# VladimirRadenkovic/Image-inpainting-and-Super-Resolution-using-Diffusion-Models-and-Conditional-Flow-Matching

Hardware: AMD Instinct MI355X
Metric: sampled images/sec (50-step, 32x32) (higher is better)
Workload: dtype bf16

## Files before the change

### image-inpainting-and-super-resolution-using-diffusion-models-and-conditional-flow-matching_amd/csrc/capi.hip

```cpp
#include <cstring>
#include <vector>

#include "capi_internal.h"

static thread_local std::string g_err;
void mi355_set_error(const std::string& msg) { g_err = msg; }

const mi355_debug_config& mi355_default_debug() {
  static const mi355_debug_config d = [] { mi355_debug_config c; mi355_debug_defaults(&c); return c; }();
  return d;
}

extern "C" {

int mi355_version(void) { return 108; }
void mi355_debug_defaults(mi355_debug_config* c) {
  if (!c) return;
  std::memset(c, 0, sizeof(*c));
  c->conv_ws = 1; c->conv_small = 15; c->conv_min_wgs = 512; c->conv_stagger = 0; c->conv_ablate = 0; c->conv_spin_limit = 1 << 22;
  c->conv_time_reps = 0; c->gn_apply_max_hw = 64; c->gn_fuse = 1; c->l2_warm = 1; c->attn_fused = 1; c->gn_epilogue = 7; c->conv_pp = 109; c->conv_edge = 15;
}
int mi355_unet_status(mi355_unet* net, int clear) {
  if (!net) { mi355_set_error("null handle"); return -1; }
  return unet_status(net, clear);
}
const char* mi355_last_error(void) { return g_err.c_str(); }

int mi355_unet_param_count(const mi355_unet_config* cfg) {
  if (!cfg) { mi355_set_error("null config"); return -1; }
  std::vector<ParamInfo> p;
  int rc = unet_enumerate_params(*cfg, p);
  return rc ? rc : (int)p.size();
}

int mi355_unet_param_info(const mi355_unet_config* cfg, int index, char* name, int name_cap, int64_t shape[4], int* ndim) {
  if (!cfg || !name || !shape || !ndim) { mi355_set_error("null argument"); return -1; }
  std::vector<ParamInfo> p;
  if (int rc = unet_enumerate_params(*cfg, p)) return rc;
  MI355_REQUIRE(index >= 0 && index < (int)p.size(), -1, "param index out of range");
  MI355_REQUIRE((int)p[index].name.size() + 1 <= name_cap, -1, "name buffer too small");
  std::strcpy(name, p[index].name.c_str());
  *ndim = (int)p[index].shape.size();
  for (int i = 0; i < 4; ++i) shape[i] = i < *ndim ? p[index].shape[i] : 1;
  return 0;
}

int64_t mi355_unet_weight_bytes(const mi355_unet_config* cfg) {
  if (!cfg) { mi355_set_error("null config"); return -1; }
  return unet_weight_bytes(*cfg);
}

int mi355_unet_create(const mi355_unet_config* cfg, const float* const* params_host, int n_params, void* dev_weights,
                      int64_t dev_weights_bytes, void* stream, mi355_unet** out) {
  if (!cfg) { mi355_set_error("null config"); return -1; }
  return unet_build(*cfg, params_host, n_params, dev_weights, dev_weights_bytes, S(stream), out);
}

void mi355_unet_destroy(mi355_unet* net) { delete net; }

int mi355_unet_forward(mi355_unet* net, const float* x, int x_channels, const float* cond, int cond_channels, const float* t,
                       float* out, int batch, void* workspace, int64_t workspace_bytes, void* stream) {
  return unet_forward(net, x, x_channels, cond, cond_channels, t, out, batch, workspace, workspace_bytes, S(stream));
}

int mi355_unet_forward_t(mi355_unet* net, const float* x, int x_channels, const float* cond, int cond_channels, float t, float* out,
                         int batch, void* workspace, int64_t workspace_bytes, void* stream) {
  MI355_REQUIRE(net && workspace && batch > 0, -1, "unet_forward_t: bad argument");
  const WsLayout l = unet_ws_layout(net, batch);
  MI355_REQUIRE((int64_t)l.total <= workspace_bytes, -2, "unet_forward_t: workspace too small");
  float* tdev = reinterpret_cast<float*>(reinterpret_cast<char*>(workspace) + l.emb2);
  if (int rc = fill_launch(tdev, t, 1, S(stream))) return rc;
  return unet_forward(net, x, x_channels, cond, cond_channels, tdev, out, batch, workspace, workspace_bytes, S(stream), uniform_t_run());
}

int mi355_unet_forward_labels(mi355_unet* net, const float* x, int x_channels, const float* cond, int cond_channels, const float* t, float t_host,
                              const int32_t* labels, float* out, int batch, void* workspace, int64_t workspace_bytes, void* stream) {
  MI355_REQUIRE(net && workspace && batch > 0, -1, "unet_forward_labels: bad argument");
  MI355_REQUIRE(!labels || net->num_classes > 0, -1, "unet_forward_labels: class labels given to a net built without num_classes");
  UnetRun run;
  run.labels = labels;
  if (!t) {
    const WsLayout l = unet_ws_layout(net, batch);
    MI355_REQUIRE((int64_t)l.total <= workspace_bytes, -2, "unet_forward_labels: workspace too small");
    float* tdev = reinterpret_cast<float*>(reinterpret_cast<char*>(workspace) + l.emb2);
    if (int rc = fill_launch(tdev, t_host, 1, S(stream))) return rc;
    t = tdev;
    run.t_uniform = 1;
  }
  return unet_forward(net, x, x_channels, cond, cond_channels, t, out, batch, workspace, workspace_bytes, S(stream), run);
}

int mi355_unet_vjp(mi355_unet* net, const float* grad_out, float* grad_x, int x_channels, int batch, void* workspace, int64_t workspace_bytes,
                   void* stream) {
  MI355_REQUIRE(net && workspace, -1, "unet_vjp: null argument");
  const int64_t engine_bytes = unet_workspace_bytes(net, batch);
  MI355_REQUIRE(workspace_bytes >= engine_bytes, -2, "unet_vjp: workspace too small");
  return unet_backward(net, grad_out, grad_x, x_channels, batch, workspace, workspace_bytes, S(stream));
}

int mi355_unet_plan_op(const mi355_unet* net, int index, int32_t fields[16]) {
  MI355_REQUIRE(net && fields, -1, "plan_op: null argument");
  if (index < 0 || index >= (int)net->ops.size()) return -1;
  const PlanOp& o = net->ops[index];
  const int32_t v[16] = {o.kind, o.src0, o.src1, o.dst, o.mode, o.ks, o.Cout, o.use_pro, o.pro_silu, o.res, o.res_mode, o.gn_site, o.heads, o.ch,
                         o.dst >= 0 ? net->tensors[o.dst].C : 0, o.dst >= 0 ? net->tensors[o.dst].H : 0};
  for (int i = 0; i < 16; ++i) fields[i] = v[i];
  return (int)net->ops.size();
}

int mi355_unet_read_tensor(const mi355_unet* net, int tensor, int gradient, float* out, int batch, void* workspace, int64_t workspace_bytes,
                           void* stream) {
  MI355_REQUIRE(net && out && workspace, -1, "read_tensor: null argument");
  MI355_REQUIRE(tensor >= 0 && tensor < (int)net->tensors.size(), -1, "read_tensor: tensor index out of range");
  MI355_REQUIRE(!gradient || net->cfg.differentiable, -4, "read_tensor: gradients exist in differentiable plans only");
  const WsView v(net, workspace, batch);
  MI355_REQUIRE((int64_t)v.l.total <= workspace_bytes, -2, "read_tensor: workspace too small");
  const PlanTensor& t = net->tensors[tensor];
  const int tstate = (!gradient && (size_t)tensor < net->tensor_state_n) ? (int)net->tensor_state[tensor].load(std::memory_order_relaxed) : 0;
  if (tstate) {
    mi355_set_error(tstate == 1
                        ? "read_tensor: the last forward did not materialise this tensor (a conv output whose only reader, a GroupNorm site, ran in the conv's "
                          "epilogue; a 1x1 skip conv that rode in the next 3x3 conv; the packed network input the first conv read from the caller's tensor): "
                          "create the handle with debug.gn_epilogue = 0, conv_small = 7, conv_edge = 3 to inspect it"
                        : "read_tensor: the last forward normalised this conv output in place (16x16 level: it holds silu(GroupNorm(.)), not the conv's result): "
                          "create the handle with debug.gn_epilogue = 0 (or 1) to inspect it");
    return MI355_ERR_UNSUPPORTED;
  }
  return unpack_nchw_launch(net->cfg.dtype, gradient ? v.grad(tensor) : v.tensor(tensor), batch, t.H * t.W, t.C, out, S(stream));
}

int mi355_unet_get_stats(const mi355_unet* net, int batch, mi355_unet_stats* out) {
  if (!net || !out) { mi355_set_error("null argument"); return -1; }
  out->launches = net->last_launches > 0 ? net->last_launches : net->launches;
  out->conv_flops = net->conv_flops * batch;
  out->attn_flops = net->attn_flops * batch;
  out->act_bytes = net->act_bytes * batch;
  out->weight_bytes = net->weight_bytes;
  return 0;
}

int mi355_unet_profile(mi355_unet* net, const float* x, int x_channels, const float* cond, int cond_channels, const float* t,
                       float* out, int batch, void* workspace, int64_t workspace_bytes, void* stream, mi355_op_profile* recs,
                       int cap) {
  MI355_REQUIRE(net && recs && cap > 0, -1, "unet_profile: bad argument");
  std::vector<mi355_op_profile> prof;
  std::vector<hipEvent_t> ev;
  UnetRun run; run.prof = &prof; run.prof_events = &ev;
  int rc = unet_forward(net, x, x_channels, cond, cond_channels, t, out, batch, workspace, workspace_bytes, S(stream), run);
  constexpr int NCAL = 17;
  hipEvent_t cal[NCAL];
  for (int i = 0; i < NCAL; ++i) { (void)hipEventCreate(&cal[i]); (void)hipEventRecord(cal[i], S(stream)); }
  hipError_t e = hipStreamSynchronize(S(stream));
  if (rc == 0 && e == hipSuccess) {
    float gap = 0.f;
    for (int i = 0; i + 1 < NCAL; ++i) { float ms = 0.f; (void)hipEventElapsedTime(&ms, cal[i], cal[i + 1]); gap += ms; }
    gap /= (float)(NCAL - 1);
    for (size_t i = 0; i + 1 < ev.size() && i < prof.size(); ++i) {
      float ms = 0.f;
      (void)hipEventElapsedTime(&ms, ev[i], ev[i + 1]);
      prof[i].ms = ms > 2.f * gap ? ms - gap : 0.5f * ms;
    }
  }
  for (int i = 0; i < NCAL; ++i) (void)hipEventDestroy(cal[i]);
  for (auto h : ev) (void)hipEventDestroy(h);
  if (rc) return rc;
  if (e != hipSuccess) { mi355_set_error(hipGetErrorString(e)); return -3; }
  const int n = (int)prof.size();
  for (int i = 0; i < n && i < cap; ++i) recs[i] = prof[i];
  return n;
}


// ... 109 lines not shown
```

### image-inpainting-and-super-resolution-using-diffusion-models-and-conditional-flow-matching_amd/csrc/conv_igemm.hip

```cpp
#include <algorithm>
#include <cstdlib>
#include <type_traits>
#include <vector>

#include "ops.h"

namespace {

constexpr int PROW = 96;

struct ConvKArgs {
  const void* src0; const void* src1;
  int C0, C1, Cin, nchunks;
  int nreal;
  int N, Hs, Ws, Hc, Wc, Ho, Wo;
  int mode, pad, stride;
  const float* pro_a; const float* pro_b; int pro_silu;
  const void* w; const float* bias; int Cout; int bn_pack;
  const float* emb; int emb_stride;
  const void* res; int res_mode; int Hr, Wr;
  void* out; int out_mode;
  float* gn_stats; int gn_slots;
  int lvw, lth, G, PW, PH, NP, tiles_x, tiles_y;
  uint32_t bytes0, bytes1, wbytes, obytes, rbytes;
// ... 611 lines not shown
}

int conv_tile_n(int Cout) {
  if (Cout % 128 == 0) return 128;
  if (Cout % 64 == 0) return 64;
  return 32;
}

static inline int chunk_of(int dtype) { return dtype == 0 ? 16 : 32; }

size_t conv_packed_weight_bytes(int dtype, int Cout, int Cin, int ks, int split) {
  const int BN = conv_tile_n(Cout), CH = chunk_of(dtype);
  const size_t nt = (Cout + BN - 1) / BN, nc = (size_t)((Cin + CH - 1) / CH) * (split ? 2 : 1);
  return nt * nc * ks * ks * (size_t)BN * 64;
}

static inline uint16_t f2bf(float f) {
  uint32_t u;
  memcpy(&u, &f, 4);
  if ((u & 0x7fffffffu) > 0x7f800000u) return (uint16_t)((u >> 16) | 0x40);
  return (uint16_t)((u + 0x7fffu + ((u >> 16) & 1u)) >> 16);
}
static inline float bf2f(uint16_t h) { uint32_t u = (uint32_t)h << 16; float f; memcpy(&f, &u, 4); return f; }

namespace {
struct PackTile {
  int dtype, BN, CH, V, esz;
  PackTile(int dtype_, int Cout) : dtype(dtype_), BN(conv_tile_n(Cout)), CH(chunk_of(dtype_)), V(CH / 4), esz(dtype_ == 0 ? 4 : 2) {}
  void store(char* tile, int row, int kl, float v) const {
    const int q = kl / V, e = kl % V;
    char* dstp = tile + row * 64 + 16 * (q ^ ((row >> 1) & 3)) + e * esz;
    if (dtype == DT_F32) memcpy(dstp, &v, 4);
    else if (dtype == DT_F16) { const _Float16 h = (_Float16)v; memcpy(dstp, &h, 2); }
    else { uint16_t h = f2bf(v); memcpy(dstp, &h, 2); }
  }
};
}

void conv_pack_weights(int dtype, const float* w, int Cout, int Cin, int ks, void* dst, int split) {
  const PackTile pk(dtype, Cout);
  const int BN = pk.BN, CH = pk.CH;
  const int nt = (Cout + BN - 1) / BN, nr = (Cin + CH - 1) / CH, nc = nr * (split && dtype == 1 ? 2 : 1), ntaps = ks * ks;
  char* out = reinterpret_cast<char*>(dst);
  memset(out, 0, conv_packed_weight_bytes(dtype, Cout, Cin, ks, split));
  for (int t = 0; t < nt; ++t)
    for (int c = 0; c < nc; ++c)
      for (int tap = 0; tap < ntaps; ++tap) {
        char* tile = out + (((size_t)t * nc + c) * ntaps + tap) * (size_t)BN * 64;
        const bool lo = c >= nr;
        for (int row = 0; row < BN; ++row) {
          const int co = t * BN + row;
          if (co >= Cout) break;
          for (int kl = 0; kl < CH; ++kl) {
            const int ci = (lo ? c - nr : c) * CH + kl;
            if (ci >= Cin) break;
            float v = w[((size_t)co * Cin + ci) * ntaps + tap];
            if (lo) v = v - bf2f(f2bf(v));
            pk.store(tile, row, kl, v);
          }
        }
      }
}

size_t conv_packed_weight_bytes_up2(int dtype, int Cout, int Cin) {
  const int BN = conv_tile_n(Cout), CH = chunk_of(dtype);
  const size_t nt = (Cout + BN - 1) / BN, nc = (size_t)((Cin + CH - 1) / CH);
  return nt * 4 * nc * 4 * (size_t)BN * 64;
}
void conv_pack_weights_up2(int dtype, const float* w, int Cout, int Cin, void* dst) {
  const PackTile pk(dtype, Cout);
  const int BN = pk.BN, CH = pk.CH;
  const int nt = (Cout + BN - 1) / BN, nc = (Cin + CH - 1) / CH;
  char* out = reinterpret_cast<char*>(dst);
  memset(out, 0, conv_packed_weight_bytes_up2(dtype, Cout, Cin));
  for (int t = 0; t < nt; ++t)
    for (int ph = 0; ph < 4; ++ph)
      for (int c = 0; c < nc; ++c)
        for (int tap = 0; tap < 4; ++tap) {
          const int pa = ph >> 1, pb = ph & 1, ty = tap >> 1, tx = tap & 1;
          char* tile = out + ((((size_t)t * 4 + ph) * nc + c) * 4 + tap) * (size_t)BN * 64;
          for (int row = 0; row < BN; ++row) {
            const int co = t * BN + row;
            if (co >= Cout) break;
            for (int kl = 0; kl < CH; ++kl) {
              const int ci = c * CH + kl;
              if (ci >= Cin) break;
              const float* w9 = w + ((size_t)co * Cin + ci) * 9;
              float v = 0.f;
              for (int ky = 0; ky < 3; ++ky)
                for (int kx = 0; kx < 3; ++kx)
                  if ((pa + ky + 1) / 2 == pa + ty && (pb + kx + 1) / 2 == pb + tx) v += w9[ky * 3 + kx];
              pk.store(tile, row, kl, v);
            }
          }
        }
}

size_t conv_packed_weight_bytes_skip(int dtype, int Cout, int Cin, int Cskip) {
  return conv_packed_weight_bytes(dtype, Cout, Cin, 3, 0) + conv_packed_weight_bytes(dtype, Cout, Cskip, 1, 0);
}
void conv_pack_weights_skip(int dtype, const float* w3, const float* w1, int Cout, int Cin, int Cskip, void* dst) {
  const size_t b3 = conv_packed_weight_bytes(dtype, Cout, Cin, 3, 0), b1 = conv_packed_weight_bytes(dtype, Cout, Cskip, 1, 0);
  std::vector<char> t3(b3), t1(b1);
  conv_pack_weights(dtype, w3, Cout, Cin, 3, t3.data(), 0);
  conv_pack_weights(dtype, w1, Cout, Cskip, 1, t1.data(), 0);
  const size_t nt = (Cout + conv_tile_n(Cout) - 1) / conv_tile_n(Cout), s3 = b3 / nt, s1 = b1 / nt;
  char* out = reinterpret_cast<char*>(dst);
  for (size_t t = 0; t < nt; ++t) {
    memcpy(out + t * (s3 + s1), t3.data() + t * s3, s3);
    memcpy(out + t * (s3 + s1) + s3, t1.data() + t * s1, s1);
  }
}

size_t conv_packed_weight_bytes_dgrad(int dtype, int Cout, int Cin, int ks, int cin_pad) { (void)Cin; return conv_packed_weight_bytes(dtype, cin_pad, Cout, ks); }
void conv_pack_weights_dgrad(int dtype, const float* w, int Cout, int Cin, int ks, int cin_pad, void* dst) {
  const int nt = ks * ks;
  std::vector<float> t((size_t)cin_pad * Cout * nt, 0.f);
  for (int co = 0; co < Cout; ++co)
    for (int ci = 0; ci < Cin; ++ci)
      for (int tap = 0; tap < nt; ++tap) t[((size_t)ci * Cout + co) * nt + (nt - 1 - tap)] = w[((size_t)co * Cin + ci) * nt + tap];
  conv_pack_weights(dtype, t.data(), cin_pad, Cout, ks, dst);
}

ConvGeom conv_geometry(const ConvDesc& d) { ConvRoute r; conv_route(d, &r); return r.geom; }

int conv_route(const ConvDesc& d, ConvRoute* r) {
  *r = ConvRoute{};
  Geo g; compute_geo(d, g);
  r->geom = ConvGeom{g.Ho, g.Wo, g.BM, g.BN, g.lds, g.groups * g.tiles_x * g.tiles_y, (d.Cout + g.BN - 1) / g.BN};
  const bool fskip = d.skip_src0 != nullptr;
  if (!fskip && !d.wsplit) {
    int rc = pp1_route(d, r);
    if (rc == 1) rc = conv1x1_route(d, r);
    if (rc == 1) rc = conv_out_route(d, r);
    if (rc == 1) rc = conv_in_route(d, r);
    if (rc <= 0) return rc;
  }
  const int CH = chunk_of(d.dtype);
  const int Cin = d.C0 + d.C1;
  MI355_REQUIRE(d.ks == 1 || d.ks == 3, -1, "conv: kernel size must be 1 or 3");
  MI355_REQUIRE(d.C0 % CH == 0 && d.C1 % CH == 0 && Cin > 0, -2, "conv: source channels must be multiples of the 64-byte chunk");
  MI355_REQUIRE(d.mode == CONV_UNIT || d.ks == 3, -1, "conv: resampling modes need a 3x3 kernel");
  MI355_REQUIRE(d.out_mode == OUT_NCHW_F32 || d.Cout % 32 == 0, -2, "conv: NHWC output needs Cout % 32 == 0 (a wave stores whole 32-channel tiles)");
  MI355_REQUIRE(d.mode != CONV_POOL2 && d.res_mode != RES_POOL2, -4, "conv: average pooling is a separate pass (affine_pool / resample), not a gather mode");
  MI355_REQUIRE(g.lds <= 160 * 1024, -4, "conv: LDS budget exceeded");
  MI355_REQUIRE(g.pit <= g.pit_t, -4, "conv: input patch too large for the staging loops");
  MI355_REQUIRE(!d.wsplit || d.dtype == DT_BF16, -1, "conv: hi / lo split weights are a bf16 mode");
  ConvKArgs a{};
  if (int rc = igemm_args(d, g, a)) return rc;
  const mi355_debug_config& K = d.knobs ? *d.knobs : mi355_default_debug();
  const bool gn_ok = d.gn_stats && d.out_mode == OUT_NHWC && g.G == 1 && d.Cout % g.BN == 0 && d.Cout % 4 == 0;
  const bool has_pro = d.pro_a != nullptr;
  const bool up_ok = d.mode == CONV_UP2 && d.w_up2 && !d.wsplit && a.res_mode == RES_NONE;
  const int pc = fskip ? -1 : pp_config(K.conv_pp, d.ks, g.G, g.bn_pack, d.out_mode, g.stride, a.nchunks, has_pro, d.pro_silu != 0, d.N, g.Ho, g.Wo, d.Cout, up_ok);
  if (pc == 2) {
    r->kernel = CONV_K_PP; r->form = 2; r->w_up2 = 1;
    r->geom.BM = 256; r->geom.BN = 256; r->geom.lds_bytes = pp::D<0>::lds_bytes(false);
    const int slots = 4 * 2 * ((d.Ws + 15) / 16) * ((d.Hs + 15) / 16);
    if (gn_ok && slots <= d.gn_slots_cap) r->gn_slots = slots;
    return 0;
  }
  if (pc >= 0) {
    r->kernel = CONV_K_PP; r->form = pc;
    r->geom.BM = pc == 0 ? 256 : 512; r->geom.BN = pc == 0 ? 256 : 128;
    r->geom.lds_bytes = pc == 0 ? pp::D<0>::lds_bytes(has_pro) : pp::D<1>::lds_bytes(has_pro);
    const bool act = pc == 0 && g.Ho == 16 && g.Wo == 16 && (d.Cout == 256 || d.Cout == 512) && a.res_mode == RES_NONE;
    if (act && d.act_out && (K.gn_epilogue & 2) && d.act_out == d.out && !d.act_raw) r->act_done = 1;
    const int slots = pc == 0 ? 2 * ((g.Wo + 15) / 16) * ((g.Ho + 15) / 16) : 4 * ((g.Wo + 31) / 32) * ((g.Ho + 15) / 16);
    if (!r->act_done && gn_ok && slots <= d.gn_slots_cap) r->gn_slots = slots;
    return 0;
  }
  if (!fskip && ws_eligible(K.conv_ws, d.ks, g.BM, g.BN, g.G, g.bn_pack, d.out_mode, g.stride, a.nchunks, d.N, g.Ho, g.Wo, d.Cout)) {
    r->kernel = CONV_K_WS;
    r->geom.BM = 256; r->geom.lds_bytes = ws::LDS_BYTES;
    const int slots = 2 * ((g.Wo + ws::VW - 1) / ws::VW) * ((g.Ho + ws::TH - 1) / ws::TH);
    if (gn_ok && slots <= d.gn_slots_cap) r->gn_slots = slots;
    return 0;
  }
  const bool act = d.act_out && (K.gn_epilogue & 1) && d.act_out != d.out, act2 = act && d.act2_out && (K.gn_epilogue & 4);
  const size_t esz = d.dtype == 0 ? 4 : 2;
  MI355_REQUIRE(!act || (size_t)d.N * g.Ho * g.Wo * (d.act_stride ? d.act_stride : d.Cout) * esz < 0xFFFF0000ull, -4,
                "conv: activated output exceeds 4 GiB (32-bit buffer offsets): run the batch in slices");
  MI355_REQUIRE(!act2 || (size_t)d.N * g.Ho * g.Wo * (d.act2_stride ? d.act2_stride : d.Cout) * esz < 0xFFFF0000ull, -4,
                "conv: activated output exceeds 4 GiB (32-bit buffer offsets): run the batch in slices");
  if (small_route(a, K.conv_small, d.ks, d.dtype, r) == 0) {
    auto cpg_ok = [&](int cpg, int coff) { return (cpg == 4 || cpg == 8 || cpg == 16) && d.Cout % cpg == 0 && coff % cpg == 0; };
    const bool ok = act && cpg_ok(d.act_cpg ? d.act_cpg : d.Cout / 32, d.act_coff) && (g.Ho != 8 || r->ksplit == 1);
    const bool ok2 = ok && act2 && cpg_ok(d.act2_cpg ? d.act2_cpg : d.Cout / 32, d.act2_coff);
    r->act_done = (ok ? 1 : 0) | (ok2 ? 2 : 0);
    return 0;
  }
  MI355_REQUIRE(!fskip, -5, "conv: no kernel carries the fused skip conv of this description (shape, batch or knobs)");
  const int slots = g.tiles_x * g.tiles_y * (g.BN == 32 ? 4 : 2);
  if (gn_ok && slots <= d.gn_slots_cap) r->gn_slots = slots;
  return 0;
}

int conv_launch(const ConvDesc& d, hipStream_t stream) { ConvRoute r; int rc = conv_route(d, &r); return rc ? rc : conv_launch(d, r, stream); }

int conv_launch(const ConvDesc& d, const ConvRoute& r, hipStream_t stream) {
  switch (r.kernel) {
    case CONV_K_1X1_PP: return pp1_launch(d, r, stream);
    case CONV_K_1X1: return conv1x1_launch(d, r, stream);
    case CONV_K_OUT: return conv_out_launch(d, r, stream);
    case CONV_K_IN: return conv_in_launch(d, r, stream);
    default: break;
  }
  Geo g; compute_geo(d, g);
  ConvKArgs a{};
  if (int rc = igemm_args(d, g, a)) return rc;
  if (r.gn_slots) { a.gn_stats = d.gn_stats; a.gn_slots = r.gn_slots; }
  if (r.w_up2) {
    MI355_REQUIRE(d.w_up2, -1, "conv: the route asks for the collapsed up-sampling weights (conv_pack_weights_up2) and the description has none");
    a.w = d.w_up2; a.wbytes = (uint32_t)conv_packed_weight_bytes_up2(d.dtype, d.Cout, d.C0 + d.C1);
  }
  const size_t esz = d.dtype == 0 ? 4 : 2;
  if (r.act_done & 1) {
    a.act_out = d.act_out; a.act_gamma = d.act_gamma; a.act_beta = d.act_beta; a.act_film = d.act_film; a.act_film_stride = d.act_film_stride;
    a.act_eps = d.act_eps; a.act_silu = d.act_silu; a.act_raw = d.act_raw;
  }
  int rc;
  if (r.kernel == CONV_K_PP) rc = dispatch_dtype(d.dtype, [&](auto t) { return launch_pp<decltype(t)>(a, r.form, stream); });
  else if (r.kernel == CONV_K_WS) rc = dispatch_dtype(d.dtype, [&](auto t) { return launch_ws<decltype(t)>(a, stream); });
  else if (r.kernel == CONV_K_SMALL) {
    if (r.act_done & 1) {
      a.act_stride = d.act_stride ? d.act_stride : d.Cout; a.act_coff = d.act_coff; a.act_cpg = d.act_cpg ? d.act_cpg : d.Cout / 32;
      a.abytes = (uint32_t)((size_t)d.N * g.Ho * g.Wo * a.act_stride * esz);
      const mi355_debug_config& K = d.knobs ? *d.knobs : mi355_default_debug();
      a.warm = (K.l2_warm & 1) ? d.warm : nullptr; a.warm_bytes = a.warm ? d.warm_bytes : 0u;
    }
    if (r.act_done & 2) {
      a.act2_out = d.act2_out; a.act2_gamma = d.act2_gamma; a.act2_beta = d.act2_beta; a.act2_silu = d.act2_silu;
      a.act2_stride = d.act2_stride ? d.act2_stride : d.Cout; a.act2_coff = d.act2_coff; a.act2_cpg = d.act2_cpg ? d.act2_cpg : d.Cout / 32;
      a.a2bytes = (uint32_t)((size_t)d.N * g.Ho * g.Wo * a.act2_stride * esz);
    }
    rc = dispatch_dtype(d.dtype, [&](auto t) { return launch_small<decltype(t)>(a, r, stream); });
  } else {
    const dim3 grid(g.groups * g.tiles_x * g.tiles_y, (d.Cout + g.BN - 1) / g.BN);
    rc = dispatch_dtype(d.dtype, [&](auto t) { return launch_cfg<decltype(t)>(a, g.BM, g.BN, d.ks, g.pit_t, grid, g.lds, stream); });
  }
  if (rc) return rc;
  MI355_CHECK_HIP(hipGetLastError());
  return 0;
}
```

### image-inpainting-and-super-resolution-using-diffusion-models-and-conditional-flow-matching_amd/csrc/conv_ws.inc.h

```cpp
#ifndef WS_ABLATE
#define WS_ABLATE 0
#endif
#ifndef WS_LSLEEP
#define WS_LSLEEP 8
#endif
#ifndef WS_CSLEEP
#define WS_CSLEEP 2
#endif
#define WS_STR2(x) #x
#define WS_STR(x) WS_STR2(x)
namespace ws {
constexpr int VW = 16, TH = 16, PW = VW + 2, PH = TH + 2, NPX = PW * PH;
constexpr int PIT = 6, FR = 64, PLANE = NPX * 64;
constexpr int AROWB = PW * 64;
constexpr int BN = 128, WTILE = BN * 64, WIT = 3 * WTILE / (256 * 16);
constexpr int CBUF = BN * 4;
constexpr int NPLANES = 3, NWBUF = 4;
constexpr size_t LDS_BYTES = NPLANES * (size_t)PLANE + NWBUF * 3 * (size_t)WTILE + 2 * CBUF + 64;
}

typedef __bf16 bf16x2_t __attribute__((ext_vector_type(2)));
template <typename T2>
__device__ __forceinline__ u32x4 ws_pro_frag(const u32x4& raw, const f32x2 (&a2)[4], const f32x2 (&b2)[4], bool silu, T2) {
  u32x4 out;
#pragma unroll
  for (int i = 0; i < 4; ++i) {
    const uint32_t w = raw[i];
    f32x2 x;
    { float xl, xh; unpack2(w, xl, xh, T2()); x = f32x2{xl, xh}; }
    f32x2 v = a2[i] * x + b2[i];
    if (silu && (WS_ABLATE & 128)) {
      const f32x2 sc = v * f32x2{-1.4426950408889634f, -1.4426950408889634f};
      const f32x2 d = sc * sc + f32x2{1.0f, 1.0f};
      v = v * (d * sc + d);
    } else if (silu) {
      const f32x2 sc = v * f32x2{-1.4426950408889634f, -1.4426950408889634f};
      const f32x2 d = f32x2{__builtin_amdgcn_exp2f(sc[0]), __builtin_amdgcn_exp2f(sc[1])} + f32x2{1.0f, 1.0f};
      v = v * f32x2{__builtin_amdgcn_rcpf(d[0]), __builtin_amdgcn_rcpf(d[1])};
    }
    out[i] = pack2(v[0], v[1], T2());
  }
  return out;
}
__device__ __forceinline__ u32x4 ws_pro_frag(const u32x4& raw, const f32x2 (&a2)[2], const f32x2 (&b2)[2], bool silu, float) {
  const f32x4 x = __builtin_bit_cast(f32x4, raw);
  f32x4 o;
#pragma unroll
  for (int j = 0; j < 4; ++j) {
    const float v = a2[j >> 1][j & 1] * x[j] + b2[j >> 1][j & 1];
    o[j] = silu ? silu_fast<false>(v) : v;
  }
  return __builtin_bit_cast(u32x4, o);
}

template <typename T, int PRO>
__global__ void __launch_bounds__(512, 2) conv3x3_ws_kernel(ConvKArgs p, int n_mt, int n_nt) {
  using namespace ws;
  using E = Elem<T>;
  constexpr int V = E::VEC, CHUNK = E::CHUNK, ESZ = sizeof(T);
  extern __shared__ __attribute__((aligned(16))) char smem[];
  char* pbuf = smem;
  char* wbuf = smem + NPLANES * PLANE;
  char* cbuf = wbuf + NWBUF * 3 * WTILE;
  uint32_t* c_prod = reinterpret_cast<uint32_t*>(cbuf + 2 * CBUF);
  uint32_t* c_cons = c_prod + 4;

  const int tid = threadIdx.x & 255, lane = threadIdx.x & 63;
  const int wave8 = __builtin_amdgcn_readfirstlane(threadIdx.x >> 6);
  const bool loader = wave8 < 4;
  const int tpi = p.tiles_x * p.tiles_y;
  const int ngr = p.nchunks * 3;
  const int ntp = ((n_mt + 7) / 8) * 8 * n_nt;
  auto decode = [&](int t, int& mt, int& nt) {
    const int per = 8 * n_nt, blk = t / per, r = t - blk * per;
    nt = r >> 3; mt = blk * 8 + (r & 7);
  };
  auto next_valid = [&](int t) {
    for (t += gridDim.x; t < ntp; t += gridDim.x) { int mt, nt; decode(t, mt, nt); if (mt < n_mt) break; }
    return t;
  };
  auto origin = [&](int mt, int& n0, int& y0, int& x0) {
    const int ng = mt / tpi, rem = mt - ng * tpi;
    const int tyi = rem / p.tiles_x, txi = rem - tyi * p.tiles_x;
    n0 = ng; y0 = tyi * TH; x0 = txi * VW;
  };
  int t_first = (int)blockIdx.x - (int)gridDim.x;
  t_first = next_valid(t_first);
  if (t_first >= ntp) return;
  if (threadIdx.x < 16) c_prod[threadIdx.x] = 0u;
  if constexpr ((WS_ABLATE & 2048) != 0) {
    for (int i = threadIdx.x; i < (NPLANES * PLANE + NWBUF * 3 * WTILE) / 16; i += 512) {
      uint32_t h = (uint32_t)i * 2654435761u + blockIdx.x * 40503u;
      u32x4 v;
#pragma unroll
      for (int k = 0; k < 4; ++k) { h ^= h >> 15; h *= 2246822519u; h ^= h >> 13; v[k] = (h & 0x807f807fu) | 0x3f003f00u; }
      *reinterpret_cast<u32x4*>(smem + (size_t)i * 16) = v;
    }
  }
  __syncthreads();
  const __attribute__((address_space(1))) uint32_t* errp = (const __attribute__((address_space(1))) uint32_t*)p.err;
#define WS_WAIT_GE_BODY(FO_) \
    const uint32_t a = (uint32_t)(uintptr_t)(const __attribute__((address_space(3))) uint32_t*)cp; \
    uint32_t v0, v1, v2, v3; int sv, spins = p.spin_limit; \
    asm volatile( \
        "1:\n\t" \
        "ds_read_b32 %[v0], %[a]\n\t" \
        "ds_read_b32 %[v1], %[a] offset:4\n\t" \
        "ds_read_b32 %[v2], %[a] offset:8\n\t" \
        "ds_read_b32 %[v3], %[a] offset:12\n\t" \
        "s_waitcnt lgkmcnt(0)\n\t" \
        "v_min_u32 %[v0], %[v0], %[v1]\n\t" \
        "v_min_u32 %[v2], %[v2], %[v3]\n\t" \
        "v_min_u32 %[v0], %[v0], %[v2]\n\t" \
        "s_nop 0\n\t" \
        "v_readfirstlane_b32 %[sv], %[v0]\n\t" \
        "s_cmp_ge_u32 %[sv], %[tg]\n\t" \
        "s_cbranch_scc1 2f\n\t" \
        "s_sub_u32 %[sp], %[sp], 1\n\t" \
        "s_cmp_eq_u32 %[sp], 0\n\t" \
        "s_cbranch_scc1 4f\n\t" \
        "ds_read_b32 %[v1], %[a] offset:%[fo]\n\t" \
        "s_waitcnt lgkmcnt(0)\n\t" \
        "v_readfirstlane_b32 %[sv], %[v1]\n\t" \
        "s_cmp_lg_u32 %[sv], 0\n\t" \
        "s_cbranch_scc1 2f\n\t" \
        "s_sleep " WS_STR(WS_LSLEEP) "\n\t" \
        "s_branch 1b\n\t" \
        "4:\n\t" \
        "s_mov_b64 exec, 1\n\t" \
        "v_mov_b32 %[v1], 1\n\t" \
        "ds_write_b32 %[a], %[v1] offset:%[fo]\n\t" \
        "s_cmp_eq_u64 %[err], 0\n\t" \
        "s_cbranch_scc1 5f\n\t" \
        "v_mov_b32 %[v0], 0\n\t" \
        "global_store_dword %[v0], %[v1], %[err] sc0 sc1\n\t" \
        "5:\n\t" \
        "s_mov_b64 exec, -1\n\t" \
        "2:" \
        : [v0] "=&v"(v0), [v1] "=&v"(v1), [v2] "=&v"(v2), [v3] "=&v"(v3), [sv] "=&s"(sv), [sp] "+s"(spins) \
        : [a] "v"(a), [tg] "s"(target), [err] "s"(errp), [fo] "i"(FO_) \
        : "scc", "memory");
  auto wait_ge_prod = [&](const uint32_t* cp, uint32_t target) { WS_WAIT_GE_BODY(48) };
  auto wait_ge_cons = [&](const uint32_t* cp, uint32_t target) { WS_WAIT_GE_BODY(32) };
#undef WS_WAIT_GE_BODY

  auto poll_issue = [&](const uint32_t* cp, uint32_t& v0, uint32_t& v1, uint32_t& v2, uint32_t& v3) {
    const u32x4 v = *reinterpret_cast<const volatile __attribute__((address_space(3))) u32x4*>((const __attribute__((address_space(3))) uint32_t*)cp);
    v0 = v[0]; v1 = v[1]; v2 = v[2]; v3 = v[3];
  };
  auto release_acquire = [&](uint32_t* mine, const uint32_t* cp, uint32_t target, uint32_t v0, uint32_t v1, uint32_t v2, uint32_t v3) {
    const uint32_t am = (uint32_t)(uintptr_t)(__attribute__((address_space(3))) uint32_t*)mine;
    const uint32_t a = (uint32_t)(uintptr_t)(const __attribute__((address_space(3))) uint32_t*)cp;
    const uint32_t one = 1u;
    int sv, spins = p.spin_limit;
    asm volatile(
        "s_mov_b64 exec, 1\n\t"
        "ds_add_u32 %[am], %[one]\n\t"
        "s_mov_b64 exec, -1\n\t"
        "s_branch 3f\n\t"
        "1:\n\t"
        "ds_read_b32 %[v0], %[a]\n\t"
        "ds_read_b32 %[v1], %[a] offset:4\n\t"
        "ds_read_b32 %[v2], %[a] offset:8\n\t"
        "ds_read_b32 %[v3], %[a] offset:12\n\t"
        "s_waitcnt lgkmcnt(0)\n\t"
        "3:\n\t"
        "v_min_u32 %[v0], %[v0], %[v1]\n\t"
        "v_min_u32 %[v2], %[v2], %[v3]\n\t"
        "v_min_u32 %[v0], %[v0], %[v2]\n\t"
        "s_nop 0\n\t"
        "v_readfirstlane_b32 %[sv], %[v0]\n\t"
        "s_cmp_ge_u32 %[sv], %[tg]\n\t"
        "s_cbranch_scc1 2f\n\t"
        "s_sub_u32 %[sp], %[sp], 1\n\t"
        "s_cmp_eq_u32 %[sp], 0\n\t"
        "s_cbranch_scc1 4f\n\t"
        "ds_read_b32 %[v1], %[a] offset:48\n\t"
        "s_waitcnt lgkmcnt(0)\n\t"
        "v_readfirstlane_b32 %[sv], %[v1]\n\t"
        "s_cmp_lg_u32 %[sv], 0\n\t"
        "s_cbranch_scc1 2f\n\t"
        "s_sleep " WS_STR(WS_CSLEEP) "\n\t"
        "s_branch 1b\n\t"
        "4:\n\t"
        "s_mov_b64 exec, 1\n\t"
        "v_mov_b32 %[v1], 1\n\t"
        "ds_write_b32 %[a], %[v1] offset:48\n\t"
        "s_cmp_eq_u64 %[err], 0\n\t"
        "s_cbranch_scc1 5f\n\t"
        "v_mov_b32 %[v0], 0\n\t"
        "global_store_dword %[v0], %[v1], %[err] sc0 sc1\n\t"
        "5:\n\t"
        "s_mov_b64 exec, -1\n\t"
        "2:"
        : [v0] "+v"(v0), [v1] "+v"(v1), [v2] "+v"(v2), [v3] "+v"(v3), [sv] "=&s"(sv), [sp] "+s"(spins)
        : [a] "v"(a), [am] "v"(am), [one] "v"(one), [tg] "s"(target), [err] "s"(errp)
        : "scc", "memory");
  };
  auto bump = [&](uint32_t* cp) {
    const uint32_t a = (uint32_t)(uintptr_t)(__attribute__((address_space(3))) uint32_t*)cp;
    const uint32_t one = 1u;
    asm volatile(
        "s_mov_b64 exec, 1\n\t"
        "ds_add_u32 %0, %1\n\t"
        "s_mov_b64 exec, -1"
        :
        : "v"(a), "v"(one)
        : "memory");
  };

  if (loader) {
    if constexpr ((WS_ABLATE & 2048) != 0) return;
    switch (p.stagger > 0 ? ((p.stagger >> 2) & 3) : 2) { case 1: __builtin_amdgcn_s_setprio(1); break; case 2: __builtin_amdgcn_s_setprio(2); break; case 3: __builtin_amdgcn_s_setprio(3); break; default: break; }
    const __amdgpu_buffer_rsrc_t rs0 = __builtin_amdgcn_make_buffer_rsrc(const_cast<void*>(p.src0), 0, p.bytes0, 0x00020000);
    const __amdgpu_buffer_rsrc_t rs1 = __builtin_amdgcn_make_buffer_rsrc(const_cast<void*>(p.src1 ? p.src1 : p.src0), 0, p.bytes1, 0x00020000);
    const __amdgpu_buffer_rsrc_t rsw = __builtin_amdgcn_make_buffer_rsrc(const_cast<void*>(p.w), 0, p.wbytes, 0x00020000);
    if constexpr (PRO == 0 && !(WS_ABLATE & 1024)) {
    constexpr int NPU = 6;
    const bool has_h1 = wave8 < 3;
    uint32_t pvo0[NPU], pvo1[NPU];
    auto piece_first_pixel = [&](int u) { const int j = 7 * (u >> 1) + 4 * (u & 1) + wave8; return j == 20 ? NPX - 16 : 16 * j; };
    auto setup = [&](int mt) {
      int n0, y0, x0;
      origin(mt, n0, y0, x0);
// ... 54 lines not shown
      wl_buf = wl_buf == NWBUF - 1 ? 0 : wl_buf + 1;
      if (++wl_row == ngr) {
        wl_row = 0;
        wl_t = next_valid(wl_t);
        if (wl_t < ntp) { int mt; decode(wl_t, mt, wl_nt); }
      }
    };
    auto wait_landed = [&](int k) {
      asm volatile("" ::: "memory");
      constexpr int WK = (WS_ABLATE & 8) ? 0 : WIT;
      if (k == 2) __builtin_amdgcn_s_waitcnt((WK + 2) | (7 << 4) | (0 << 8));
      else if (k == 1) __builtin_amdgcn_s_waitcnt((WK + 1) | (7 << 4) | (0 << 8));
      else __builtin_amdgcn_s_waitcnt(WK | (7 << 4) | (0 << 8));
    };
    int R = 0;
    auto acquire_free = [&]() {
      if (R >= NWBUF - 1) wait_ge_cons(c_cons, (uint32_t)(R - (NWBUF - 2)));
    };
    f32x4 cv_b = f32x4{0.f, 0.f, 0.f, 0.f}, cv_e = f32x4{0.f, 0.f, 0.f, 0.f};
    int cst_par = 0;
    auto cinit_load = [&](int t) {
      int mt, nt, n0, y0, x0;
      decode(t, mt, nt);
      origin(mt, n0, y0, x0);
      const int co = min(nt * BN + (tid & 31) * 4, p.Cout - 4);
      const float* dummy = reinterpret_cast<const float*>(p.w);
      cv_b = *reinterpret_cast<const f32x4*>(p.bias ? p.bias + co : dummy);
      cv_e = *reinterpret_cast<const f32x4*>(p.emb ? p.emb + (size_t)n0 * p.emb_stride + co : dummy);
    };
    auto cinit_commit = [&]() {
      if (tid < 32) {
        f32x4 v;
#pragma unroll
        for (int j = 0; j < 4; ++j) v[j] = (p.bias ? cv_b[j] : 0.0f) + (p.emb ? cv_e[j] : 0.0f);
        *reinterpret_cast<f32x4*>(cbuf + cst_par * CBUF + tid * 16) = v;
      }
      cst_par ^= 1;
    };
    STAMP_DECL
    cinit_load(t_first);
    cinit_commit();
    (void)issue_pieces(IC<0>()); (void)issue_pieces(IC<1>()); (void)issue_pieces(IC<2>());
    pt_advance();
    dma_w();
    STAMP(0)
    for (int t = t_first; t < ntp;) {
      const int t_next = next_valid(t);
      for (int c = 0; c < p.nchunks; ++c) {
        const bool last_c = c + 1 == p.nchunks && t_next < ntp;
        auto tail = [&](int k) {
          dma_w();
          STAMP(3)
          wait_landed(k);
          STAMP(1)
          if (!((p.ablate & 32) && R == 5)) bump(c_prod + wave8);
          ++R;
          acquire_free();
          STAMP(4)
        };
        if (last_c) cinit_load(t_next);
        const int k0 = issue_pieces(IC<0>());
        tail(k0);
        const int k1 = issue_pieces(IC<1>());
        tail(k1);
        const int k2 = issue_pieces(IC<2>());
        pt_advance();
        if (last_c) cinit_commit();
        tail(k2);
      }
      t = t_next;
    }
    __builtin_amdgcn_s_waitcnt(0 | (7 << 4) | (15 << 8));
    STAMP_FLUSH
    } else {
    const int fq = tid & 3, frow = tid >> 2;
    const bool pok5 = (lane >> 2) < 4;
    const bool pro = PRO && !(p.ablate & 2);
    int pdst[PIT];
#pragma unroll
    for (int u = 0; u < PIT; ++u) {
      const int i = u < 5 ? frow + u * FR : 320 + (lane >> 2);
      const int py = (int)(((float)i + 0.5f) * (1.0f / (float)PW)), px = i - py * PW;
      pdst[u] = i * 64 + 16 * (fq ^ ((px >> 1) & 3));
    }
    int xw = 0;
    uint32_t woff[WIT];
#pragma unroll
    for (int i = 0; i < WIT; ++i) woff[i] = (i * 256 + tid) * 16;

    uint32_t voff0[PIT], voff1[PIT], vmask_ld = 0; int n0_ld = 0;
    auto setup = [&](int mt) {
      int n0, y0, x0;
      origin(mt, n0, y0, x0);
      n0_ld = n0; vmask_ld = 0;
      const int cy0 = y0 - 1, cx0 = x0 - 1;
#pragma unroll
      for (int u = 0; u < PIT; ++u) {
        const int i = u < 5 ? frow + u * FR : 320 + (lane >> 2);
        int s = -1;
        if (u < 5 || pok5) {
          const int py = (int)(((float)i + 0.5f) * (1.0f / (float)PW)), px = i - py * PW;
          const int cy = cy0 + py, cx = cx0 + px;
          if (cy >= 0 && cy < p.Hc && cx >= 0 && cx < p.Wc) {
            if (p.mode == CONV_UP2) s = (n0 * p.Hs + (cy >> 1)) * p.Ws + (cx >> 1);
            else s = (n0 * p.Hs + cy) * p.Ws + cx;
          }
        }
        voff0[u] = s >= 0 ? (uint32_t)s * (uint32_t)(p.C0 * ESZ) + fq * 16 : p.bytes0;
        voff1[u] = s >= 0 ? (uint32_t)s * (uint32_t)(p.C1 * ESZ) + fq * 16 : p.bytes1;
        if (s >= 0) vmask_ld |= 1u << u;
      }
    };
    int ld_t = t_first, ld_c = 0;
    { int mt, nt; decode(ld_t, mt, nt); setup(mt); }
    auto ld_advance = [&]() {
      if (++ld_c == p.nchunks) {
        ld_c = 0;
        ld_t = next_valid(ld_t);
        if (ld_t < ntp) { int mt, nt; decode(ld_t, mt, nt); setup(mt); }
      }
    };
    u32x4 raw[PIT] = {};
    f32x2 pa[V / 2] = {}, pb[V / 2] = {}, pan[V / 2] = {}, pbn[V / 2] = {};
    auto issue_frag = [&](auto uc) {
      constexpr int u = decltype(uc)::value;
      const int cb = src_chunk(p, ld_c) * CHUNK;
      const bool first = cb < p.C0;
      if constexpr (!(WS_ABLATE & 16)) raw[u] = buf_load16(first ? rs0 : rs1, first ? voff0[u] : voff1[u], (first ? cb : cb - p.C0) * ESZ);
    };
    auto issue_ab = [&]() {
      if constexpr (PRO) {
        const float* ap = p.pro_a + (size_t)n0_ld * p.Cin + src_chunk(p, ld_c) * CHUNK + fq * V;
        const float* bp = p.pro_b + (size_t)n0_ld * p.Cin + src_chunk(p, ld_c) * CHUNK + fq * V;
#pragma unroll
        for (int j = 0; j < V / 2; ++j) { pan[j] = *reinterpret_cast<const f32x2*>(ap + 2 * j); pbn[j] = *reinterpret_cast<const f32x2*>(bp + 2 * j); }
      }
    };
    auto take_ab = [&]() {
#pragma unroll
      for (int j = 0; j < V / 2; ++j) { pa[j] = pan[j]; pb[j] = pbn[j]; }
    };
    auto commit_frag = [&](auto uc, int plane, uint32_t mask) {
      constexpr int u = decltype(uc)::value;
      if constexpr (u == 5) { if (wave8 != xw) return; }
      u32x4 outv = raw[u];
      if (pro) {
        outv = ws_pro_frag(raw[u], pa, pb, PRO == 2, T());
        if (!((mask >> u) & 1u)) outv = u32x4{0u, 0u, 0u, 0u};
      }
      if (u < 5 || pok5) *reinterpret_cast<u32x4*>(pbuf + plane * PLANE + pdst[u]) = outv;
    };

    int wl_t = t_first, wl_row = 0, wl_nt, wl_buf = 0;
    { int mt; decode(wl_t, mt, wl_nt); }
    auto dma_w = [&]() {
      const uint32_t so = ((uint32_t)wl_nt * p.nchunks * 9 + (uint32_t)wl_row * 3) * WTILE;
      if constexpr (!(WS_ABLATE & 8)) {
        char* dst = wbuf + wl_buf * (3 * WTILE) + wave8 * 1024;
#pragma unroll
        for (int i = 0; i < WIT; ++i)
          __builtin_amdgcn_raw_ptr_buffer_load_lds(rsw, (__attribute__((address_space(3))) void*)(dst + i * 4096), 16, woff[i], so, 0, 0);
      }
      wl_buf = wl_buf == NWBUF - 1 ? 0 : wl_buf + 1;
      if (++wl_row == ngr) {
        wl_row = 0;
        wl_t = next_valid(wl_t);
        if (wl_t < ntp) { int mt; decode(wl_t, mt, wl_nt); }
      }
    };
    auto wait_landed = [&]() {
      asm volatile("" ::: "memory");
      __builtin_amdgcn_s_waitcnt(8 | (7 << 4) | (0 << 8));
    };
    int R = 0;
    auto acquire_free = [&]() {
      if (R >= NWBUF - 1) wait_ge_cons(c_cons, (uint32_t)(R - (NWBUF - 2)));
    };

    f32x4 cv_b = f32x4{0.f, 0.f, 0.f, 0.f}, cv_e = f32x4{0.f, 0.f, 0.f, 0.f};
    int cst_par = 0;
    auto cinit_load = [&](int t) {
      int mt, nt, n0, y0, x0;
      decode(t, mt, nt);
      origin(mt, n0, y0, x0);
      const int co = min(nt * BN + (tid & 31) * 4, p.Cout - 4);
      const float* dummy = reinterpret_cast<const float*>(p.w);
      cv_b = *reinterpret_cast<const f32x4*>(p.bias ? p.bias + co : dummy);
      cv_e = *reinterpret_cast<const f32x4*>(p.emb ? p.emb + (size_t)n0 * p.emb_stride + co : dummy);
    };
    auto cinit_commit = [&]() {
      const float fb = p.bias ? 1.0f : 0.0f, fe = p.emb ? 1.0f : 0.0f;
      if (tid < 32) {
        f32x4 v;
#pragma unroll
        for (int j = 0; j < 4; ++j) v[j] = (p.bias ? cv_b[j] : 0.0f) + (p.emb ? cv_e[j] : 0.0f);
        *reinterpret_cast<f32x4*>(cbuf + cst_par * CBUF + tid * 16) = v;
      }
      (void)fb; (void)fe;
      cst_par ^= 1;
    };
    cinit_load(t_first);
    STAMP_DECL
    issue_frag(IC<0>()); issue_frag(IC<1>()); issue_frag(IC<2>()); issue_frag(IC<3>()); issue_frag(IC<4>()); issue_frag(IC<5>());
    issue_ab();
    dma_w();
    uint32_t vmask_cm = vmask_ld;
    take_ab();
    ld_advance();
    issue_ab();
    commit_frag(IC<0>(), 0, vmask_cm); issue_frag(IC<0>());
    commit_frag(IC<1>(), 0, vmask_cm); issue_frag(IC<1>());
    commit_frag(IC<2>(), 0, vmask_cm); issue_frag(IC<2>());
    commit_frag(IC<3>(), 0, vmask_cm); issue_frag(IC<3>());
    cinit_commit();

    STAMP(0)
    int plane = 0;
    for (int t = t_first; t < ntp;) {
      const int t_next = next_valid(t);
      auto body = [&](int c) {
        bool nx_ok = true;
        auto tail = [&]() {
          dma_w();
          STAMP(3)
          wait_landed();
          STAMP(1)
          if (!((p.ablate & 32) && R == 5)) bump(c_prod + wave8);
          ++R;
          acquire_free();
          STAMP(4)
        };
        cinit_load(t_next < ntp ? t_next : t);
        commit_frag(IC<4>(), plane, vmask_cm); issue_frag(IC<4>());
        commit_frag(IC<5>(), plane, vmask_cm); issue_frag(IC<5>());
        xw = (xw + 1) & 3;
        STAMP(2)
        tail();
        if (c + 1 == p.nchunks) {
          nx_ok = t_next < ntp;
          vmask_cm = vmask_ld;
        }
        take_ab();
        ld_advance();
        issue_ab();
        plane = plane == NPLANES - 1 ? 0 : plane + 1;
        if (nx_ok) commit_frag(IC<0>(), plane, vmask_cm);
        issue_frag(IC<0>());
        if (nx_ok) commit_frag(IC<1>(), plane, vmask_cm);
        issue_frag(IC<1>());
        STAMP(2)
        tail();
        if (nx_ok) commit_frag(IC<2>(), plane, vmask_cm);
        issue_frag(IC<2>());
        if (nx_ok) commit_frag(IC<3>(), plane, vmask_cm);
        issue_frag(IC<3>());
        if (c + 1 == p.nchunks && nx_ok) cinit_commit();
        STAMP(2)
        tail();
      };
      for (int c = 0; c < p.nchunks; c += 2) { body(c); body(c + 1); }
      t = t_next;
    }
    __builtin_amdgcn_s_waitcnt(0 | (7 << 4) | (15 << 8));
    STAMP_FLUSH
    }
  } else {
    switch (p.stagger > 0 ? (p.stagger & 3) : 1) { case 1: __builtin_amdgcn_s_setprio(1); break; case 2: __builtin_amdgcn_s_setprio(2); break; case 3: __builtin_amdgcn_s_setprio(3); break; default: break; }
    const int wave = wave8 - 4;
    const int wm = wave >> 1, wn = wave & 1;
    const int lr = lane & 15, lq = lane >> 4;
    int a_cur[3];
#pragma unroll
    for (int kx = 0; kx < 3; ++kx) a_cur[kx] = (wm * 8 * PW + lr + kx) * 64 + 16 * (lq ^ (((lr + kx) >> 1) & 3));
    int b_cur = (wn * 64 + lr) * 64 + 16 * (lq ^ ((lr >> 1) & 3));
    const __amdgpu_buffer_rsrc_t rso = __builtin_amdgcn_make_buffer_rsrc(p.out, 0, (p.ablate & 1) ? 0u : p.obytes, 0x00020000);
    const __amdgpu_buffer_rsrc_t rsr = __builtin_amdgcn_make_buffer_rsrc(const_cast<void*>(p.res ? p.res : p.out), 0, p.rbytes, 0x00020000);
    constexpr bool PAIR = E::DTYPE == 1;
    constexpr int NI = 4, NP2 = PAIR ? NI / 2 : NI, PSTEP = PAIR ? 32 : 16;

    f32x4 acc[8][NI];
    u32x4 af[2][4], bf[2][4];
    typedef float f32x16_t __attribute__((ext_vector_type(16)));
    f32x16_t accb[8];
    f32x4 cin[NI];
    int cpar = 0;
    auto read_cinit = [&]() {
#pragma unroll
      for (int ni = 0; ni < NI; ++ni) cin[ni] = *reinterpret_cast<const f32x4*>(cbuf + cpar * CBUF + (wn * 64 + ni * 16 + lq * 4) * 4);
      cpar ^= 1;
    };
    STAMP_DECL
    CLK_DECL
    int ky = 0, plane = 0, sel = 0;
    uint32_t rowc = 0;
    uint32_t pq0 = 0, pq1 = 0, pq2 = 0, pq3 = 0;
    const bool gate512 = p.N > 0;
    auto advance_row = [&]() {
      int bstep = 3 * WTILE, astep = AROWB;
      if (sel == NWBUF - 1) { sel = 0; bstep = -(NWBUF - 1) * 3 * WTILE; } else ++sel;
      if (++ky == 3) {
        ky = 0;
        if (plane == NPLANES - 1) { plane = 0; astep = -(NPLANES - 1) * PLANE - 2 * AROWB; } else { ++plane; astep = PLANE - 2 * AROWB; }
      }
#pragma unroll
      for (int kx = 0; kx < 3; ++kx) a_cur[kx] += astep;
      b_cur += bstep;
    };
    auto read_a = [&](auto bufc, auto halfc, auto kxc) {
      constexpr int buf = decltype(bufc)::value, half = decltype(halfc)::value, kx = decltype(kxc)::value;
      if constexpr (WS_ABLATE & 4) return;
      if constexpr (WS_ABLATE & 512) { if (gate512) return; }
#pragma unroll
      for (int j = 0; j < 4; ++j) af[buf][j] = *reinterpret_cast<const u32x4*>(pbuf + a_cur[kx] + (half * 4 + j) * AROWB);
    };
    auto read_b = [&](auto bufc, auto kxc) {
      constexpr int buf = decltype(bufc)::value, kx = decltype(kxc)::value;
      if constexpr (WS_ABLATE & 4) return;
      if constexpr (WS_ABLATE & 512) { if (gate512) return; }
#pragma unroll
      for (int ni = 0; ni < NI; ++ni) bf[buf][ni] = *reinterpret_cast<const u32x4*>(wbuf + b_cur + kx * WTILE + ni * 1024);
    };
    auto step = [&](auto Rc, auto sc, auto zeroc, bool more_rows) {
      constexpr int R = decltype(Rc)::value, s = decltype(sc)::value;
      constexpr bool ZERO = decltype(zeroc)::value != 0;
      constexpr int half = s & 1, kx = s >> 1, bpar = (R + kx) & 1;
      if constexpr (s < 5) {
        constexpr int s1 = s + 1, half1 = s1 & 1, kx1 = s1 >> 1;
        read_a(IC<half1>(), IC<half1>(), IC<kx1>());
        if constexpr (half1 == 0) read_b(IC<(R + kx1) & 1>(), IC<kx1>());
        if constexpr (s == 4 && !(WS_ABLATE & 2048)) poll_issue(c_prod, pq0, pq1, pq2, pq3);
      } else {
        if (more_rows) {
          STAMP(6)
          if constexpr (!(WS_ABLATE & 2048)) release_acquire(c_cons + wave, c_prod, rowc + 2u, pq0, pq1, pq2, pq3);
          ++rowc;
          STAMP(5)
          advance_row();
          read_a(IC<0>(), IC<0>(), IC<0>());
          read_b(IC<(R + 1) & 1>(), IC<0>());
        }
      }
      __builtin_amdgcn_sched_barrier(0);
      if constexpr ((WS_ABLATE & 256) != 0 && Elem<T>::DTYPE == 1) {
#pragma unroll
        for (int j = 0; j < 4; ++j)
#pragma unroll
          for (int h2 = 0; h2 < 2; ++h2) {
            if constexpr (ZERO) accb[half * 4 + j] = f32x16_t{};
            accb[half * 4 + j] = __builtin_amdgcn_mfma_f32_32x32x16_bf16(__builtin_bit_cast(bf16x8, bf[bpar][2 * h2]), __builtin_bit_cast(bf16x8, af[half][j]), accb[half * 4 + j], 0, 0, 0);
          }
      } else if constexpr (!(WS_ABLATE & 4)) {
#pragma unroll
        for (int j = 0; j < 4; ++j)
#pragma unroll
          for (int ni = 0; ni < NI; ++ni) {
            if constexpr (ZERO) acc[half * 4 + j][ni] = cin[ni];
            mma16(acc[half * 4 + j][ni], bf[bpar][ni], af[half][j], T());
          }
      } else if constexpr (ZERO) {
#pragma unroll
        for (int j = 0; j < 4; ++j)
#pragma unroll
          for (int ni = 0; ni < NI; ++ni) acc[half * 4 + j][ni] = cin[ni];
      }
      __builtin_amdgcn_sched_barrier(0);
    };

    if constexpr (!(WS_ABLATE & 2048)) wait_ge_prod(c_prod, 1u);
    STAMP(5)
    read_a(IC<0>(), IC<0>(), IC<0>());
    read_b(IC<0>(), IC<0>());
    for (int t = t_first; t < ntp;) {
      const int t_next = next_valid(t);
      int mt, nt, n0, y0, x0;
      decode(t, mt, nt);
      origin(mt, n0, y0, x0);
      const int co_w = nt * BN + wn * 64 + 4 * lq;
      for (int r = 0; r < ngr; r += 2) {
        const bool last_pair = r + 2 >= ngr;
        if (r == 0) { read_cinit(); step(IC<0>(), IC<0>(), IC<1>(), true); step(IC<0>(), IC<1>(), IC<1>(), true); }
        else { step(IC<0>(), IC<0>(), IC<0>(), true); step(IC<0>(), IC<1>(), IC<0>(), true); }
        step(IC<0>(), IC<2>(), IC<0>(), true); step(IC<0>(), IC<3>(), IC<0>(), true);
        step(IC<0>(), IC<4>(), IC<0>(), true); step(IC<0>(), IC<5>(), IC<0>(), true);
        step(IC<1>(), IC<0>(), IC<0>(), true); step(IC<1>(), IC<1>(), IC<0>(), true);
        step(IC<1>(), IC<2>(), IC<0>(), true); step(IC<1>(), IC<3>(), IC<0>(), true);
        step(IC<1>(), IC<4>(), IC<0>(), true); step(IC<1>(), IC<5>(), IC<0>(), !last_pair);
      }
      if (t_next < ntp) bump(c_cons + wave);
      if constexpr ((WS_ABLATE & 256) != 0) {
#pragma unroll
        for (int mi = 0; mi < 8; ++mi)
#pragma unroll
          for (int ni = 0; ni < NI; ++ni) acc[mi][ni] = f32x4{accb[mi][4 * ni], accb[mi][4 * ni + 1], accb[mi][4 * ni + 2], accb[mi][4 * ni + 3]};
      }
      STAMP(6)
      const int co_s = PAIR ? nt * BN + wn * 64 + (lq & 1) * 16 + (lq >> 1) * 8 : co_w;
      GnPartial<NI> gp;
      const bool do_gn = p.gn_stats != nullptr;
      const bool gn_mask = ((p.Wo | p.Ho) & 15) != 0;
      auto epi_half = [&](auto hc, auto resc, auto gnc) {
        constexpr int h = decltype(hc)::value, GNM = decltype(gnc)::value;
        constexpr bool HAS_RES = decltype(resc)::value != 0;
        uint32_t ovo[4], rvo[4];
        float vm[4];
#pragma unroll
        for (int j = 0; j < 4; ++j) {
          const int y = y0 + wm * 8 + h * 4 + j, x = x0 + lr;
          const bool ok = y < p.Ho && x < p.Wo && co_s < p.Cout;
          vm[j] = (y < p.Ho && x < p.Wo) ? 1.f : 0.f;
          const uint32_t opix = (uint32_t)((n0 * p.Ho + y) * p.Wo + x);
          ovo[j] = ok ? (opix * (uint32_t)p.Cout + (uint32_t)co_s) * ESZ : p.obytes;
          uint32_t rpix = opix;
          if (p.res_mode == RES_UP2) rpix = (uint32_t)((n0 * p.Hr + (y >> 1)) * p.Wr + (x >> 1));
          rvo[j] = (ok && HAS_RES) ? (rpix * (uint32_t)p.Cout + (uint32_t)co_s) * ESZ : p.rbytes;
        }
        u32x4 rr[4][NP2];
        if constexpr (HAS_RES) {
#pragma unroll
          for (int j = 0; j < 4; ++j)
#pragma unroll
            for (int k = 0; k < NP2; ++k)
              rr[j][k] = __builtin_bit_cast(u32x4, __builtin_amdgcn_raw_buffer_load_b128(rsr, rvo[j] + k * PSTEP * ESZ, 0, 0));
        }
#pragma unroll
        for (int j = 0; j < 4; ++j) {
          const int mi = h * 4 + j;
          if constexpr (!PAIR) {
#pragma unroll
            for (int ni = 0; ni < NI; ++ni) {
              f32x4 o = acc[mi][ni];
              if constexpr (HAS_RES) {
                const f32x4 tt = __builtin_bit_cast(f32x4, rr[j][ni]);
                o = f32x4{o[0] + tt[0], o[1] + tt[1], o[2] + tt[2], o[3] + tt[3]};
              }
              if constexpr (GNM != 0) gp.add(ni, o[0], o[1], o[2], o[3], GNM == 2, vm[j]);
              __builtin_amdgcn_raw_buffer_store_b128(__builtin_bit_cast(u32x4, o), rso, ovo[j] + ni * 16 * ESZ, 0, 0);
            }
          } else {
#pragma unroll
            for (int k = 0; k < NP2; ++k) {
              float ra[4] = {0.f, 0.f, 0.f, 0.f}, rb[4] = {0.f, 0.f, 0.f, 0.f};
              if constexpr (HAS_RES) {
                const auto s0 = __builtin_amdgcn_permlane16_swap(rr[j][k][0], rr[j][k][2], false, false);
                const auto s1 = __builtin_amdgcn_permlane16_swap(rr[j][k][1], rr[j][k][3], false, false);
                const uint32_t xa[2] = {s0[0], s1[0]}, xb[2] = {s0[1], s1[1]};
#pragma unroll
                for (int q = 0; q < 2; ++q) {
                  unpack2(xa[q], ra[2 * q], ra[2 * q + 1], T());
                  unpack2(xb[q], rb[2 * q], rb[2 * q + 1], T());
                }
              }
              float va[4], vb[4];
#pragma unroll
              for (int q = 0; q < 4; ++q) {
                va[q] = HAS_RES ? acc[mi][2 * k][q] + ra[q] : acc[mi][2 * k][q];
                vb[q] = HAS_RES ? acc[mi][2 * k + 1][q] + rb[q] : acc[mi][2 * k + 1][q];
              }
              if constexpr (GNM != 0) {
                gp.add(2 * k, va[0], va[1], va[2], va[3], GNM == 2, vm[j]);
                gp.add(2 * k + 1, vb[0], vb[1], vb[2], vb[3], GNM == 2, vm[j]);
              }
              const u32x2 pa2 = pack4(va, T()), pb2 = pack4(vb, T());
              const auto w0 = __builtin_amdgcn_permlane16_swap(pa2[0], pb2[0], false, false);
              const auto w1 = __builtin_amdgcn_permlane16_swap(pa2[1], pb2[1], false, false);
              __builtin_amdgcn_raw_buffer_store_b128(u32x4{w0[0], w1[0], w0[1], w1[1]}, rso, ovo[j] + k * PSTEP * ESZ, 0, 0);
            }
          }
        }
      };
      auto epi = [&](auto resc, auto gnc) { epi_half(IC<0>(), resc, gnc); epi_half(IC<1>(), resc, gnc); };
      if (p.res_mode != RES_NONE) {
        if (!do_gn) epi(IC<1>(), IC<0>()); else if (!gn_mask) epi(IC<1>(), IC<1>()); else epi(IC<1>(), IC<2>());
      } else {
        if (!do_gn) epi(IC<0>(), IC<0>()); else if (!gn_mask) epi(IC<0>(), IC<1>()); else epi(IC<0>(), IC<2>());
      }
      if (do_gn) {
        const int rem = mt - n0 * tpi;
        gp.store(p.gn_stats + (((size_t)n0 * p.gn_slots + rem * 2 + wm) * (size_t)(p.Cout >> 2) + ((nt * BN + wn * 64) >> 2)) * 2, lq, lr);
      }
      STAMP(7)
      if (t_next < ntp) {
        if constexpr (!(WS_ABLATE & 2048)) wait_ge_prod(c_prod, rowc + 2u);
        ++rowc;
        advance_row();
        read_a(IC<0>(), IC<0>(), IC<0>());
        read_b(IC<0>(), IC<0>());
      }
      t = t_next;
    }
    STAMP_FLUSH
    CLK_FLUSH
  }
}

static int ws_num_cus() {
  static const int ncu = [] { int dev = 0, n = 256; if (hipGetDevice(&dev) == hipSuccess) { hipDeviceProp_t pr; if (hipGetDeviceProperties(&pr, dev) == hipSuccess) n = pr.multiProcessorCount; } return n; }();
  return ncu;
}
static bool ws_eligible(int enabled, int ks, int BM, int BN, int G, int bn_pack, int out_mode, int stride, int nchunks, int N, int Ho, int Wo, int Cout) {
  if (!enabled || ks != 3 || BM != 128 || BN != 128 || G != 1 || bn_pack != 128 || out_mode != OUT_NHWC) return false;
  if (stride != 1 || nchunks < 2 || (nchunks & 1)) return false;
  if (Wo < ws::VW || Ho < ws::TH) return false;
  const int n_mt = N * ((Wo + ws::VW - 1) / ws::VW) * ((Ho + ws::TH - 1) / ws::TH), n_nt = (Cout + 127) / 128;
  return n_mt * n_nt >= ws_num_cus();
}

template <typename T>
int launch_ws(ConvKArgs a, hipStream_t s) {
  a.lvw = 4; a.lth = 4; a.PW = ws::PW; a.PH = ws::PH; a.NP = ws::NPX;
  a.tiles_x = (a.Wo + ws::VW - 1) / ws::VW; a.tiles_y = (a.Ho + ws::TH - 1) / ws::TH;
  const int n_mt = a.N * a.tiles_x * a.tiles_y, n_nt = (a.Cout + 127) / 128;
  const int ncu = ws_num_cus();
  using KernT = void (*)(ConvKArgs, int, int);
  KernT kern = !a.pro_a ? (KernT)conv3x3_ws_kernel<T, 0> : (a.pro_silu ? (KernT)conv3x3_ws_kernel<T, 2> : (KernT)conv3x3_ws_kernel<T, 1>);
  int rc;
  if (!a.pro_a) rc = mi355_allow_big_lds(conv3x3_ws_kernel<T, 0>, "conv3x3 (persistent)");
  else if (a.pro_silu) rc = mi355_allow_big_lds(conv3x3_ws_kernel<T, 2>, "conv3x3 (persistent)");
  else rc = mi355_allow_big_lds(conv3x3_ws_kernel<T, 1>, "conv3x3 (persistent)");
  if (rc) return rc;
  const int ntp = ((n_mt + 7) / 8) * 8 * n_nt;
  const int grid = ntp < ncu ? ntp : ncu;
  hipLaunchKernelGGL(kern, dim3(grid), dim3(512), ws::LDS_BYTES, s, a, n_mt, n_nt);
  return 0;
}
```

### image-inpainting-and-super-resolution-using-diffusion-models-and-conditional-flow-matching_amd/csrc/unet_engine.hip

```cpp
#include "unet_engine.h"

#include <algorithm>
#include <cstring>
#include <map>

namespace {

inline size_t align_up(size_t v, size_t a) { return (v + a - 1) / a * a; }

enum BlockKind { BLK_CONV_IN, BLK_RES, BLK_ATTN, BLK_RESAMPLE_CONV, BLK_RESAMPLE, BLK_OUT };
struct Block {
  std::string prefix;
  int kind, cin, cout;
  int dir = 0;
  bool upsample = false;
  bool push = false, pop = false;
};
std::vector<Block> unet_blocks(const mi355_unet_config& cfg) {
  const int mc = cfg.model_channels, nl = cfg.n_channel_mult;
  auto has_attn = [&](int ds) { for (int i = 0; i < cfg.n_attention_ds; ++i) if (cfg.attention_ds[i] == ds) return true; return false; };
  std::vector<Block> out;
  auto add = [&](const std::string& prefix, int kind, int cin, int cout, int dir = 0) -> Block& {
    Block b; b.prefix = prefix; b.kind = kind; b.cin = cin; b.cout = cout; b.dir = dir;
    out.push_back(b);
// ... 66 lines not shown
    if (cfg.num_head_channels == -1) {
      int nh = (upsample && cfg.num_heads_upsample != -1) ? cfg.num_heads_upsample : cfg.num_heads;
      return nh;
    }
    return ch / cfg.num_head_channels;
  }

  size_t alloc(size_t bytes) {
    size_t o = cursor;
    cursor = align_up(cursor + bytes, 256);
    if (!dry) blob.resize(cursor, 0);
    return o;
  }
  const float* P(const std::string& name, std::vector<int64_t> expect) {
    auto it = pidx.find(name);
    if (it == pidx.end()) { err = "missing parameter " + name; return nullptr; }
    if (params[it->second].shape != expect) { err = "shape mismatch for " + name; return nullptr; }
    return dry ? nullptr : host[it->second];
  }
  size_t put_f32(const std::string& name, std::vector<int64_t> shape) {
    const float* p = P(name, shape);
    int64_t n = 1; for (auto s : shape) n *= s;
    size_t o = alloc((size_t)n * 4);
    if (!dry && p) memcpy(blob.data() + o, p, (size_t)n * 4);
    return o;
  }
  size_t put_conv(const std::string& name, int Cout, int Cin, int ks, bool conv1d) {
    std::vector<int64_t> shape = conv1d ? std::vector<int64_t>{Cout, Cin, 1} : std::vector<int64_t>{Cout, Cin, ks, ks};
    const float* p = P(name, shape);
    size_t bytes = conv_packed_weight_bytes(dtype, Cout, Cin, ks, net->wsplit);
    size_t o = alloc(bytes);
    if (!dry && p) conv_pack_weights(dtype, p, Cout, Cin, ks, blob.data() + o, net->wsplit);
    net->weight_bytes += (double)Cout * Cin * ks * ks * esz;
    return o;
  }
  size_t put_linear_t(const std::string& name, int J, int K) {
    const float* p = P(name, {J, K});
    size_t o = alloc((size_t)J * K * 4);
    if (!dry && p) {
      float* d = reinterpret_cast<float*>(blob.data() + o);
      for (int j = 0; j < J; ++j) for (int k = 0; k < K; ++k) d[(size_t)k * J + j] = p[(size_t)j * K + k];
    }
    return o;
  }

  int tensor(int C, int H, int W) {
    PlanTensor t{C, H, W, false, net->act_elems_per_image};
    net->act_elems_per_image += align_up((size_t)C * H * W, 128);
    net->tensors.push_back(t);
    return (int)net->tensors.size() - 1;
  }
  const PlanTensor& T(int id) const { return net->tensors[id]; }

  int add_gn(int s0, int s1, const std::string& wname, const std::string& bname, int film_off, int apply_silu, bool may_apply = true) {
    const int max_hw = net->knobs.gn_apply_max_hw;
    const int C = T(s0).C + (s1 >= 0 ? T(s1).C : 0);
    PlanOp op; op.kind = OP_GN; op.src0 = s0; op.src1 = s1;
    op.gamma_off = put_f32(wname, {C}); op.beta_off = put_f32(bname, {C}); op.film_emb_off = film_off;
    if (cfg.differentiable) {
      op.gn_site = last_site = (int)net->site_C.size();
      net->site_C.push_back(C);
      net->site_off.push_back(net->site_floats_per_image);
      net->site_floats_per_image += (size_t)2 * C + 64;
    } else if (may_apply && T(s0).H * T(s0).W <= max_hw) { op.dst = tensor(C, T(s0).H, T(s0).W); op.pro_silu = apply_silu; }
    else {
      const int fuse = net->knobs.gn_fuse;
      const int C1 = s1 >= 0 ? T(s1).C : 0;
      if (fuse && (C / 32) % 4 == 0 && T(s0).C % 4 == 0 && C1 % 4 == 0) {
        op.fin_ok = 1;
        for (int s : {s0, s1}) {
          if (s < 0 || net->tensors[s].stats_cap) continue;
          PlanTensor& t = net->tensors[s];
          t.stats_cap = 4 * ((t.H * t.W + 63) / 64) + 8;
          t.stats_off_per_image = net->stats_floats_per_image;
          net->stats_floats_per_image += (size_t)t.stats_cap * (t.C / 4) * 2;
        }
      }
    }
    net->ops.push_back(op);
    if (C > net->max_gn_c) net->max_gn_c = C;
    return op.dst;
  }
  int add_conv(const std::string& prefix, int s0, int s1, int Cin_logical, int Cout, int ks, int mode, bool conv1d, int use_pro,
               int pro_silu, int emb_off, int res, int res_mode, int out_mode) {
    PlanOp op; op.kind = OP_CONV; op.src0 = s0; op.src1 = s1; op.mode = mode; op.ks = ks; op.Cout = Cout;
    op.w_off = put_conv(prefix + ".weight", Cout, Cin_logical, ks, conv1d);
    op.bias_off = put_f32(prefix + ".bias", {Cout});
    op.use_pro = use_pro; op.pro_silu = pro_silu; op.emb_off = emb_off; op.res = res; op.res_mode = res_mode; op.out_mode = out_mode;
    const int cin_t = T(s0).C + (s1 >= 0 ? T(s1).C : 0);
    if (mode == CONV_UP2 && ks == 3 && !conv1d && !use_pro && res < 0 && out_mode == OUT_NHWC && !cfg.differentiable && !net->wsplit && (net->knobs.conv_pp & 64) &&
        Cout % 256 == 0 && cin_t == Cin_logical && T(s0).H >= 16 && T(s0).W >= 16) {
      const float* pw = P(prefix + ".weight", {Cout, Cin_logical, ks, ks});
      op.has_wu = 1; op.wu_off = alloc(conv_packed_weight_bytes_up2(dtype, Cout, Cin_logical));
      if (!dry && pw) conv_pack_weights_up2(dtype, pw, Cout, Cin_logical, blob.data() + op.wu_off);
    }
    int Ho = T(s0).H, Wo = T(s0).W;
    if (mode == CONV_UP2) { Ho *= 2; Wo *= 2; }
    else if (mode == CONV_POOL2) { Ho /= 2; Wo /= 2; }
    else if (mode == CONV_STRIDE2) { Ho = (Ho - 1) / 2 + 1; Wo = (Wo - 1) / 2 + 1; }
    op.dst = out_mode == OUT_NHWC ? tensor(Cout, Ho, Wo) : -1;
    if (cfg.differentiable) {
      if (use_pro) op.gn_site = last_site;
      op.cin_pad = (int)align_up(T(s0).C + (s1 >= 0 ? T(s1).C : 0), 32);
      const float* pw = P(prefix + ".weight", conv1d ? std::vector<int64_t>{Cout, Cin_logical, 1} : std::vector<int64_t>{Cout, Cin_logical, ks, ks});
      op.wT_off = alloc(conv_packed_weight_bytes_dgrad(dtype, Cout, Cin_logical, ks, op.cin_pad));
      if (!dry && pw) conv_pack_weights_dgrad(dtype, pw, Cout, Cin_logical, ks, op.cin_pad, blob.data() + op.wT_off);
      const size_t hw_dgrad = mode == CONV_UP2 ? (size_t)Ho * Wo : (size_t)T(s0).H * T(s0).W;
      net->bwd_du_elems = std::max(net->bwd_du_elems, hw_dgrad * op.cin_pad);
      if (mode == CONV_STRIDE2) net->bwd_z_elems = std::max(net->bwd_z_elems, (size_t)T(s0).H * T(s0).W * Cout);
      net->bwd_tmp_elems = std::max(net->bwd_tmp_elems, (size_t)T(s0).H * T(s0).W * op.cin_pad);
    }
    net->ops.push_back(op);
    const double in_elems = (double)(T(s0).C + (s1 >= 0 ? T(s1).C : 0)) * T(s0).H * T(s0).W;
    net->conv_flops += 2.0 * Ho * Wo * (double)Cout * Cin_logical * ks * ks;
    net->act_bytes += (in_elems + (double)Cout * Ho * Wo) * esz;
    return op.dst;
  }

  int res_block(const std::string& p, int s0, int s1, int cin, int cout, bool up, bool down) {
    const bool film = cfg.use_scale_shift_norm != 0;
    const int ew = film ? 2 * cout : cout;
    const int eoff = emb_total;
    emb_parts.push_back({p + ".emb_layers.1", eoff, ew});
    emb_total += ew;
    P(p + ".emb_layers.1.weight", {ew, 4 * cfg.model_channels});
    P(p + ".emb_layers.1.bias", {ew});
    const int y1 = add_gn(s0, s1, p + ".in_layers.0.weight", p + ".in_layers.0.bias", -1, 1, !down);
    int h1;
    int res = s0, res_mode = up ? RES_UP2 : RES_SAME;
    if (down) {
      if (s1 >= 0) { err = "ResBlock(down) over a channel concat is not supported"; return -1; }
      PlanOp op; op.kind = OP_POOLAFF; op.src0 = s0; op.pro_silu = 1;
      op.dst = tensor(T(s0).C, T(s0).H / 2, T(s0).W / 2);
      if (cfg.differentiable) { op.gn_site = last_site; net->bwd_tmp_elems = std::max(net->bwd_tmp_elems, (size_t)T(s0).H * T(s0).W * T(s0).C); }
      net->ops.push_back(op);
      h1 = add_conv(p + ".in_layers.2", op.dst, -1, cin, cout, 3, CONV_UNIT, false, 0, 0, film ? -1 : eoff, -1, RES_NONE, OUT_NHWC);
      res = resample(s0, CONV_POOL2);
    } else {
      h1 = y1 >= 0 ? add_conv(p + ".in_layers.2", y1, -1, cin, cout, 3, up ? CONV_UP2 : CONV_UNIT, false, 0, 0, film ? -1 : eoff, -1, RES_NONE, OUT_NHWC)
                   : add_conv(p + ".in_layers.2", s0, s1, cin, cout, 3, up ? CONV_UP2 : CONV_UNIT, false, 1, 1, film ? -1 : eoff, -1, RES_NONE, OUT_NHWC);
    }
    const int y2 = add_gn(h1, -1, p + ".out_layers.0.weight", p + ".out_layers.0.bias", film ? eoff : -1, 1);
    if (cin != cout) {
      if (up || down) { err = "ResBlock(up/down) with a channel change is not supported"; return -1; }
      auto it = pidx.find(p + ".skip_connection.weight");
      const int sks = (it != pidx.end() && params[it->second].shape.size() == 4) ? (int)params[it->second].shape[3] : 1;
      res = add_conv(p + ".skip_connection", s0, s1, cin, cout, sks, CONV_UNIT, false, 0, 0, -1, -1, RES_NONE, OUT_NHWC);
      res_mode = RES_SAME;
    } else if (s1 >= 0) {
      err = "identity skip over a channel concat is not supported";
      return -1;
    }
    const int skip_idx = cin != cout ? (int)net->ops.size() - 1 : -1;
    if (y2 >= 0) {
      const int out = add_conv(p + ".out_layers.3", y2, -1, cout, cout, 3, CONV_UNIT, false, 0, 0, -1, res, res_mode, OUT_NHWC);
      if (out >= 0 && skip_idx >= 0 && net->ops[skip_idx].ks == 1 && !cfg.differentiable && !net->wsplit && cout % 128 == 0) {
        const int conv2_idx = (int)net->ops.size() - 1;
        PlanOp& c2 = net->ops[conv2_idx];
        const float* w3 = P(p + ".out_layers.3.weight", {cout, cout, 3, 3});
        const float* w1 = P(p + ".skip_connection.weight", {cout, cin, 1, 1});
        const float* b3 = P(p + ".out_layers.3.bias", {cout});
        const float* b1 = P(p + ".skip_connection.bias", {cout});
        c2.wf_off = alloc(conv_packed_weight_bytes_skip(dtype, cout, cout, cin));
        c2.bf_off = alloc((size_t)cout * 4);
        if (!dry && w3 && w1 && b3 && b1) {
          conv_pack_weights_skip(dtype, w3, w1, cout, cout, cin, blob.data() + c2.wf_off);
          float* bs = reinterpret_cast<float*>(blob.data() + c2.bf_off);
          for (int i = 0; i < cout; ++i) bs[i] = b3[i] + b1[i];
        }
        c2.skip_op = skip_idx;
        net->ops[skip_idx].carrier = conv2_idx;
      }
      return out;
    }
    return add_conv(p + ".out_layers.3", h1, -1, cout, cout, 3, CONV_UNIT, false, 1, 1, -1, res, res_mode, OUT_NHWC);
  }

  int attn_block(const std::string& p, int x, int C, int heads) {
    if (heads <= 0 || C % heads != 0) { err = "attention: bad head count"; return -1; }
    const int ch = C / heads;
    {
      bool ok = false;
      for (int v : {32, 64, 96, 128, 192, 256, 384, 512}) ok = ok || ch == v;
      if (!ok) { err = "attention: head channels must be one of 32, 64, 96, 128, 192, 256, 384, 512 (got " + std::to_string(ch) + ")"; return -1; }
    }
    if (cfg.differentiable && ch > 256) {
      err = "attention: differentiable plans support head channels up to 256 (got " + std::to_string(ch) + ")";
      return -1;
    }
    const int yn = add_gn(x, -1, p + ".norm.weight", p + ".norm.bias", -1, 0);
    const double Tn_ = (double)T(x).H * T(x).W;
    if (yn < 0 && !cfg.differentiable && !net->wsplit && attn_fused_eligible(dtype, T(x).H * T(x).W, C, heads, ch, &net->knobs)) {
      PlanOp op; op.kind = OP_ATTN_FUSED; op.src0 = x; op.heads = heads; op.ch = ch; op.Cout = 3 * C;
      op.w_off = put_conv(p + ".qkv.weight", 3 * C, C, 1, true);
      op.bias_off = put_f32(p + ".qkv.bias", {3 * C});
      op.dst = tensor(C, T(x).H, T(x).W);
      net->ops.push_back(op);
      net->conv_flops += 2.0 * Tn_ * 3.0 * C * C;
      net->attn_flops += 4.0 * Tn_ * Tn_ * C;
      net->act_bytes += (2.0 * C * Tn_) * esz;
      return add_conv(p + ".proj_out", op.dst, -1, C, C, 1, CONV_UNIT, true, 0, 0, -1, x, RES_SAME, OUT_NHWC);
    }
    const int qkv = yn >= 0 ? add_conv(p + ".qkv", yn, -1, C, 3 * C, 1, CONV_UNIT, true, 0, 0, -1, -1, RES_NONE, OUT_NHWC)
                            : add_conv(p + ".qkv", x, -1, C, 3 * C, 1, CONV_UNIT, true, 1, 0, -1, -1, RES_NONE, OUT_NHWC);
    PlanOp op; op.kind = OP_ATTN; op.src0 = qkv; op.heads = heads; op.ch = ch;
    op.dst = tensor(C, T(x).H, T(x).W);
    net->ops.push_back(op);
    if (cfg.differentiable) net->bwd_ld_floats = std::max(net->bwd_ld_floats, (size_t)2 * heads * T(x).H * T(x).W);
    const double Tn = (double)T(x).H * T(x).W;
    net->attn_flops += 4.0 * Tn * Tn * C;
    net->act_bytes += (4.0 * C * Tn) * esz;
    return add_conv(p + ".proj_out", op.dst, -1, C, C, 1, CONV_UNIT, true, 0, 0, -1, x, RES_SAME, OUT_NHWC);
  }

  int resample(int x, int mode) {
    PlanOp op; op.kind = OP_RESAMPLE; op.src0 = x; op.mode = mode;
    const int Ho = mode == CONV_UP2 ? T(x).H * 2 : T(x).H / 2, Wo = mode == CONV_UP2 ? T(x).W * 2 : T(x).W / 2;
    op.dst = tensor(T(x).C, Ho, Wo);
    net->ops.push_back(op);
    return op.dst;
  }

  int walk() {
    const int mc = cfg.model_channels, S = cfg.image_size;
    net->in_pad = (int)align_up(cfg.in_channels, CH);
    net->te_w0 = put_linear_t("time_embed.0.weight", 4 * mc, mc);
    net->te_b0 = put_f32("time_embed.0.bias", {4 * mc});
    net->te_w2 = put_linear_t("time_embed.2.weight", 4 * mc, 4 * mc);
    net->te_b2 = put_f32("time_embed.2.bias", {4 * mc});
    if (cfg.num_classes > 0) {
      net->num_classes = cfg.num_classes;
      net->label_w = put_f32("label_emb.weight", {cfg.num_classes, 4 * mc});
    }
    net->in_tensor = tensor(net->in_pad, S, S);
    int h = net->in_tensor;
    std::vector<int> hs;
    for (const Block& b : unet_blocks(cfg)) {
      int skip = -1;
      if (b.pop) { skip = hs.back(); hs.pop_back(); }
      switch (b.kind) {
        case BLK_CONV_IN: h = add_conv(b.prefix, h, -1, b.cin, b.cout, 3, CONV_UNIT, false, 0, 0, -1, -1, RES_NONE, OUT_NHWC); break;
        case BLK_RES: h = res_block(b.prefix, h, skip, b.cin, b.cout, b.dir > 0, b.dir < 0); break;
        case BLK_ATTN: h = attn_block(b.prefix, h, b.cout, heads_for(b.cout, b.upsample)); break;
        case BLK_RESAMPLE_CONV:
          h = add_conv(b.prefix, h, -1, b.cin, b.cout, 3, b.dir > 0 ? CONV_UP2 : CONV_STRIDE2, false, 0, 0, -1, -1, RES_NONE, OUT_NHWC);
          break;
        case BLK_RESAMPLE: h = resample(h, b.dir > 0 ? CONV_UP2 : CONV_POOL2); break;
        case BLK_OUT:
          add_gn(h, -1, b.prefix + ".0.weight", b.prefix + ".0.bias", -1, 1, false);
          add_conv(b.prefix + ".2", h, -1, b.cin, b.cout, 3, CONV_UNIT, false, 1, 1, -1, -1, RES_NONE, OUT_NCHW_F32);
          break;
      }
      if (!err.empty()) return -1;
      if (b.push) hs.push_back(h);
    }
    const int K = 4 * mc;
    net->emb_total = emb_total;
    net->emb_w = alloc((size_t)K * emb_total * 4);
    net->emb_b = alloc((size_t)emb_total * 4);
    if (!dry) {
      float* W = reinterpret_cast<float*>(blob.data() + net->emb_w);
      float* Bv = reinterpret_cast<float*>(blob.data() + net->emb_b);
      for (auto& e : emb_parts) {
        const float* w = host[pidx[e.name + ".weight"]];
        const float* b = host[pidx[e.name + ".bias"]];
        for (int j = 0; j < e.width; ++j) {
          Bv[e.off + j] = b[j];
          for (int k = 0; k < K; ++k) W[(size_t)k * emb_total + e.off + j] = w[(size_t)j * K + k];
        }
      }
    }
    net->conv_flops += 2.0 * (double)K * emb_total + 2.0 * (double)mc * K + 2.0 * (double)K * K;
    net->out_channels = cfg.out_channels;
    net->launches = 5 + (int64_t)net->ops.size();
    return 0;
  }
};

int check_cfg(const mi355_unet_config& c) {
  MI355_REQUIRE(c.dtype == MI355_F32 || c.dtype == MI355_BF16 || c.dtype == MI355_BF16X2 || c.dtype == MI355_F16, -1,
                "unet: dtype must be MI355_F32, MI355_BF16, MI355_BF16X2 or MI355_F16");
  MI355_REQUIRE(!((c.dtype == MI355_BF16X2 || c.dtype == MI355_F16) && c.differentiable), -4, "unet: MI355_BF16X2 / MI355_F16 plans have no backward pass");
  MI355_REQUIRE(c.n_channel_mult >= 1 && c.n_channel_mult <= 8 && c.n_attention_ds >= 0 && c.n_attention_ds <= 8, -1, "unet: bad config arrays");
  MI355_REQUIRE(c.model_channels % 32 == 0 && c.model_channels > 0, -4, "unet: model_channels must be a multiple of 32 (GroupNorm32 + 64-byte channel chunks)");
  MI355_REQUIRE(c.in_channels > 0 && c.in_channels <= 32 && c.out_channels > 0 && c.out_channels <= 32, -4, "unet: in/out channels must be in 1..32");
  MI355_REQUIRE(c.image_size > 0 && c.num_res_blocks > 0, -1, "unet: bad sizes");
  MI355_REQUIRE(c.num_classes >= 0, -1, "unet: num_classes must be >= 0 (0: no label embedding)");
  return 0;
}

}

int unet_enumerate_params(const mi355_unet_config& cfg, std::vector<ParamInfo>& out) {
  if (int rc = check_cfg(cfg)) return rc;
  out.clear();
  const int mc = cfg.model_channels, E = 4 * mc;
  auto add = [&](const std::string& n, std::vector<int64_t> s) { out.push_back({n, s}); };
  auto conv = [&](const std::string& p, int co, int ci, int k) { add(p + ".weight", {co, ci, k, k}); add(p + ".bias", {co}); };
  auto res = [&](const std::string& p, int cin, int cout) {
    add(p + ".in_layers.0.weight", {cin}); add(p + ".in_layers.0.bias", {cin});
    conv(p + ".in_layers.2", cout, cin, 3);
    const int ew = cfg.use_scale_shift_norm ? 2 * cout : cout;
    add(p + ".emb_layers.1.weight", {ew, E}); add(p + ".emb_layers.1.bias", {ew});
    add(p + ".out_layers.0.weight", {cout}); add(p + ".out_layers.0.bias", {cout});
    conv(p + ".out_layers.3", cout, cout, 3);
    if (cin != cout) conv(p + ".skip_connection", cout, cin, 1);
  };
  auto attn = [&](const std::string& p, int C) {
    add(p + ".norm.weight", {C}); add(p + ".norm.bias", {C});
    add(p + ".qkv.weight", {3 * C, C, 1}); add(p + ".qkv.bias", {3 * C});
    add(p + ".proj_out.weight", {C, C, 1}); add(p + ".proj_out.bias", {C});
  };
  add("time_embed.0.weight", {E, mc}); add("time_embed.0.bias", {E});
  add("time_embed.2.weight", {E, E}); add("time_embed.2.bias", {E});
  if (cfg.num_classes > 0) add("label_emb.weight", {cfg.num_classes, E});
  for (const Block& b : unet_blocks(cfg)) {
    switch (b.kind) {
      case BLK_CONV_IN: case BLK_RESAMPLE_CONV: conv(b.prefix, b.cout, b.cin, 3); break;
      case BLK_RES: res(b.prefix, b.cin, b.cout); break;
      case BLK_ATTN: attn(b.prefix, b.cout); break;
      case BLK_RESAMPLE: break;
      case BLK_OUT: add(b.prefix + ".0.weight", {b.cin}); add(b.prefix + ".0.bias", {b.cin}); conv(b.prefix + ".2", b.cout, b.cin, 3); break;
    }
  }
  return 0;
}

static bool apply_site(const PlanOp& o) { return o.kind == OP_GN && o.dst >= 0 && o.gn_site < 0; }
// ... 499 lines not shown
```

### image-inpainting-and-super-resolution-using-diffusion-models-and-conditional-flow-matching_amd/mi355/_lib.py

```python
from __future__ import annotations

import ctypes as C
import os
import subprocess
import threading

_HERE = os.path.dirname(os.path.abspath(__file__))
CSRC = os.path.join(os.path.dirname(_HERE), "csrc")
LIB_PATH = os.environ.get("MI355_SAMPLER_LIB") or os.path.join(os.path.dirname(os.path.dirname(_HERE)), "lib", "libmi355_sampler.so")

MI355_F16 = 3
MI355_F32, MI355_BF16, MI355_BF16X2 = 0, 1, 2
DDPM_PRIOR, DDPM_AMORTIZED, DDPM_REPLACEMENT, DDIM = 0, 1, 2, 3


class MI355BackendError(RuntimeError):
    pass


class DebugConfigC(C.Structure):
    _fields_ = [("conv_ws", C.c_int32), ("conv_small", C.c_int32), ("conv_min_wgs", C.c_int32), ("conv_stagger", C.c_int32),
                ("conv_ablate", C.c_int32), ("conv_spin_limit", C.c_int32), ("conv_time_reps", C.c_int32), ("gn_apply_max_hw", C.c_int32),
                ("gn_fuse", C.c_int32), ("l2_warm", C.c_int32), ("attn_fused", C.c_int32), ("gn_epilogue", C.c_int32), ("conv_pp", C.c_int32), ("conv_edge", C.c_int32), ("sampler_graph", C.c_int32), ("reserved", C.c_int32 * 1)]


_DEBUG_ENV = {"MI355_CONV_WS": "conv_ws", "MI355_CONV_SMALL": "conv_small", "MI355_CONV_MINWG": "conv_min_wgs", "MI355_CONV_STAGGER": "conv_stagger",
              "MI355_CONV_ABLATE": "conv_ablate", "MI355_CONV_SPIN": "conv_spin_limit", "MI355_CONV_TIME": "conv_time_reps",
              "MI355_GN_APPLY_MAXHW": "gn_apply_max_hw", "MI355_GN_FUSE": "gn_fuse", "MI355_L2_WARM": "l2_warm", "MI355_ATTN_FUSE": "attn_fused",
              "MI355_GN_EPILOGUE": "gn_epilogue", "MI355_CONV_PP": "conv_pp", "MI355_CONV_EDGE": "conv_edge", "MI355_SAMPLER_GRAPH": "sampler_graph"}


def debug_config(**overrides) -> "DebugConfigC":
    d = DebugConfigC()
    lib().mi355_debug_defaults(C.byref(d))
    for env, field in _DEBUG_ENV.items():
        if os.environ.get(env, "") != "":
            setattr(d, field, int(os.environ[env]))
    for k, v in overrides.items():
        if k not in dict((f[0], 1) for f in DebugConfigC._fields_):
            raise KeyError(k)
        setattr(d, k, int(v))
    return d


class UNetConfigC(C.Structure):
    _fields_ = [
        ("image_size", C.c_int32), ("in_channels", C.c_int32), ("model_channels", C.c_int32),
        ("out_channels", C.c_int32), ("num_res_blocks", C.c_int32), ("n_attention_ds", C.c_int32),
        ("attention_ds", C.c_int32 * 8), ("n_channel_mult", C.c_int32), ("channel_mult", C.c_int32 * 8),
        ("conv_resample", C.c_int32), ("num_heads", C.c_int32), ("num_head_channels", C.c_int32),
        ("num_heads_upsample", C.c_int32), ("use_scale_shift_norm", C.c_int32), ("resblock_updown", C.c_int32),
        ("use_new_attention_order", C.c_int32), ("dtype", C.c_int32), ("differentiable", C.c_int32),
        ("debug", C.POINTER(DebugConfigC)), ("num_classes", C.c_int32),
    ]


class ConvExtrasC(C.Structure):
    _fields_ = [("skip_x0", C.c_void_p), ("skip_x1", C.c_void_p), ("skip_c0", C.c_int32), ("skip_c1", C.c_int32),
                ("skip_w_host", C.c_void_p), ("skip_bias_host", C.c_void_p),
                ("act_out", C.c_void_p * 2), ("act_gamma", C.c_void_p * 2), ("act_beta", C.c_void_p * 2),
                ("act_ctotal", C.c_int32 * 2), ("act_coff", C.c_int32 * 2), ("act_silu", C.c_int32 * 2),
                ("act_film", C.c_void_p), ("act_done", C.c_int32), ("skip_done", C.c_int32), ("route", C.c_int32 * 4)]


class UNetStatsC(C.Structure):
    _fields_ = [("launches", C.c_int64), ("conv_flops", C.c_double), ("attn_flops", C.c_double),
                ("act_bytes", C.c_double), ("weight_bytes", C.c_double)]


class OpProfileC(C.Structure):
    _fields_ = [("kind", C.c_int32), ("ks", C.c_int32), ("cin", C.c_int32), ("cout", C.c_int32), ("h", C.c_int32),
                ("w", C.c_int32), ("tile_m", C.c_int32), ("tile_n", C.c_int32), ("ms", C.c_float), ("flops", C.c_double),
                ("bytes", C.c_double)]


_FP = C.POINTER(C.c_float)


class DDPMTablesC(C.Structure):
    _fields_ = [("Ns", C.c_int32)] + [(n, _FP) for n in (
        "sqrt_recip_alphas_cumprod", "sqrt_recipm1_alphas_cumprod", "posterior_mean_coef1", "posterior_mean_coef2",
        "posterior_log_variance_clipped", "sqrt_alphas_cumprod", "sqrt_one_minus_alphas_cumprod",
        "recip_sqrt_m1_alphas_cumprod", "alphas_cumprod_prev")]


class DDPMOptionsC(C.Structure):
    _fields_ = [("mode", C.c_int32), ("n_corrector", C.c_int32), ("delta", C.c_float), ("tmin", C.c_float),
                ("tmax", C.c_float), ("start_fraction", C.c_float), ("noise_condition", C.c_int32),
                ("pad_value", C.c_float), ("none_value", C.c_float), ("cond_is_none", C.c_int32), ("seed", C.c_uint64)]


_VP, _I, _I64, _F, _U64 = C.c_void_p, C.c_int, C.c_int64, C.c_float, C.c_uint64

SIGNATURES = {
    "mi355_version": (_I, []),
    "mi355_last_error": (C.c_char_p, []),
    "mi355_debug_defaults": (None, [C.POINTER(DebugConfigC)]),
    "mi355_unet_status": (_I, [_VP, _I]),
    "mi355_unet_param_count": (_I, [C.POINTER(UNetConfigC)]),
    "mi355_unet_param_info": (_I, [C.POINTER(UNetConfigC), _I, C.c_char_p, _I, C.POINTER(C.c_int64), C.POINTER(C.c_int)]),
    "mi355_unet_weight_bytes": (_I64, [C.POINTER(UNetConfigC)]),
    "mi355_unet_create": (_I, [C.POINTER(UNetConfigC), C.POINTER(_VP), _I, _VP, _I64, _VP, C.POINTER(_VP)]),
    "mi355_unet_destroy": (None, [_VP]),
    "mi355_unet_workspace_bytes": (_I64, [_VP, _I]),
    "mi355_unet_forward": (_I, [_VP, _VP, _I, _VP, _I, _VP, _VP, _I, _VP, _I64, _VP]),
    "mi355_unet_forward_t": (_I, [_VP, _VP, _I, _VP, _I, _F, _VP, _I, _VP, _I64, _VP]),
    "mi355_unet_forward_labels": (_I, [_VP, _VP, _I, _VP, _I, _VP, _F, _VP, _VP, _I, _VP, _I64, _VP]),
    "mi355_unet_vjp": (_I, [_VP, _VP, _VP, _I, _I, _VP, _I64, _VP]),
    "mi355_unet_plan_op": (_I, [_VP, _I, C.POINTER(C.c_int32)]),
    "mi355_unet_read_tensor": (_I, [_VP, _I, _I, _VP, _I, _VP, _I64, _VP]),
    "mi355_unet_get_stats": (_I, [_VP, _I, C.POINTER(UNetStatsC)]),
    "mi355_unet_profile": (_I, [_VP, _VP, _I, _VP, _I, _VP, _VP, _I, _VP, _I64, _VP, C.POINTER(OpProfileC), _I]),
    "mi355_cfm_euler_sample": (_I, [_VP, _VP, _I, _VP, _I, _I, _FP, _I, _VP, _VP, _I, _VP, _I64, _VP]),
    "mi355_cfm_euler_sample_labels": (_I, [_VP, _VP, _I, _VP, _I, _I, _VP, _FP, _I, _VP, _VP, _I, _VP, _I64, _VP]),
    "mi355_cfm_rk_workspace_bytes": (_I64, [_VP, _I, _I]),
    "mi355_cfm_rk_sample": (_I, [_VP, _VP, _I, _VP, _I, _VP, _FP, _I, _I, _FP, _FP, _FP, _VP, _VP, _I, _VP, _I64, _VP]),
    "mi355_cfg_workspace_bytes": (_I64, [_VP, _I, _I]),
    "mi355_cfm_cfg_sample": (_I, [_VP, _VP, _I, _VP, _I, _F, _VP, _I, _F, _VP, _FP, _I, _I, _FP, _FP, _FP, _VP, _VP, _I, _VP, _I64, _VP]),
    "mi355_ddpm_cfg_workspace_bytes": (_I64, [_VP, _I]),
    "mi355_ddpm_cfg_sample": (_I, [_VP, _VP, _I, _VP, _VP, _I, _F, _VP, C.POINTER(DDPMTablesC), C.POINTER(DDPMOptionsC), _VP, _I64, _I, _VP, _I64,
                                   _VP]),
    "mi355_cfm_recon_workspace_bytes": (_I64, [_VP, _I, _I, _I]),
    "mi355_cfm_recon_sample": (_I, [_VP, _VP, _I, _VP, _FP, _I, _VP, _I, _F, _I, _I, _FP, _I, _I, _VP, _U64, _VP, _VP, _VP, _I, _VP, _I64, _VP]),
    "mi355_sf2m_euler_sample": (_I, [_VP, _VP, _VP, _I, _VP, _FP, _I, _F, _I, _VP, _U64, C.POINTER(C.c_int32), _FP, _I, _VP, _I, _VP, _I64,
                                     _VP, _I64, _VP]),
    "mi355_ddpm_sample": (_I, [_VP, _VP, _I, _VP, C.POINTER(DDPMTablesC), C.POINTER(DDPMOptionsC), _VP, _I64, _I, _VP, _I64, _VP]),
    "mi355_timestep_embedding": (_I, [_VP, _I, _I, _F, _VP, _VP]),
    "mi355_groupnorm": (_I, [_VP, _VP, _VP, _VP, _I, _I, _I, _I, _F, _I, _VP]),
    "mi355_euler_step": (_I, [_VP, _VP, _F, _I64, _VP]),
    "mi355_sde_euler_step": (_I, [_VP, _VP, _VP, _F, _F, _F, _VP, _F, _VP, _I, _U64, _U64, _VP, _F, _I64, _VP]),
    "mi355_ddpm_step": (_I, [_VP, _VP, _VP, _F, _F, _F, _F, _F, _I, _U64, _U64, _I64, _VP]),
    "mi355_corrector_step": (_I, [_VP, _VP, _VP, _F, _F, _F, _F, _F, _I, _U64, _U64, _I64, _VP]),
    "mi355_ddim_step": (_I, [_VP, _VP, _F, _F, _F, _I64, _VP]),
    "mi355_replace_mask": (_I, [_VP, _VP, _VP, _F, _I, _F, _F, _I, _U64, _U64, _I64, _VP]),
    "mi355_guidance_seed": (_I, [_VP, _VP, _VP, _F, _F, _I, _F, _I64, _VP, _VP, _I64, _VP]),
    "mi355_guidance_update": (_I, [_VP, _VP, _VP, _F, _I, _VP, _I64, _VP]),
    "mi355_lowres_seed": (_I, [_VP, _VP, _VP, _F, _F, _I, _I, _I, _I, _I, _I, _VP, _VP, _VP, _VP, _VP]),
    "mi355_clip": (_I, [_VP, _F, _F, _I64, _VP]),
    "mi355_ema_update": (_I, [_VP, _VP, _F, _F, _I64, _VP]),
    "mi355_mse_per_sample": (_I, [_VP, _VP, _VP, C.c_int, _I64, _VP]),
    "mi355_lincomb_per_sample": (_I, [_VP, _VP, _VP, _VP, _VP, _I, _I64, _VP]),
    "mi355_resize_bilinear": (_I, [_VP, _VP, _I64, _I, _I, _I, _I, _VP]),
    "mi355_paint_patch": (_I, [_VP, _VP, _VP, _I, _F, _I, _VP, _I, _I, _I, _I, _VP]),
    "mi355_quantize_u8": (_I, [_VP, _VP, _I64, _VP]),
    "mi355_to_unit_range": (_I, [_VP, _VP, _I64, _VP]),
    "mi355_randn": (_I, [_VP, _U64, _U64, _I64, _VP]),
    "mi355_rk_combine": (_I, [_VP, _VP, _VP, _VP, _VP, _VP, _VP, _VP, _VP, _FP, _I, _I64, _VP]),
    "mi355_rk_stage": (_I, [_VP, _VP, C.POINTER(_VP), _FP, _I, _I64, _VP, _VP, _VP]),
    "mi355_cfg_stage": (_I, [_VP, _VP, C.POINTER(_VP), _FP, _I, _I64, _F, _VP, _I64, _I, _VP, _VP, _VP]),
    "mi355_ddpm_cfg_step": (_I, [_VP, _VP, _VP, _F, _VP, _I64, _F, _F, _F, _F, _F, _I, _U64, _U64, _I64, _VP]),
    "mi355_ddim_cfg_step": (_I, [_VP, _VP, _F, _VP, _I64, _F, _F, _F, _I64, _VP]),
    "mi355_rk_sqnorm": (_I, [_VP, _VP, _VP, _VP, _F, _F, _I64, _VP, _VP]),
    "mi355_rk_interp": (_I, [_VP, _VP, _VP, _VP, _VP, _VP, _F, _F, _I64, _VP]),
    "mi355_op_workspace_bytes": (_I64, [_I, _I, _I]),
    "mi355_box_probe_workspace_bytes": (_I64, []),
    "mi355_box_probe": (_I, [_I, _VP, _I64, _VP, _FP, _FP, _FP]),
    "mi355_box_probe_hbm_workspace_bytes": (_I64, []),
    "mi355_box_probe_hbm": (_I, [_I, _VP, _I64, _VP, _FP, _FP]),
    "mi355_conv2d": (_I, [_VP, _VP, _I, _FP, _FP, _VP, _I, _I, _I, _I, _I, _I, _I, _I, _VP, _VP, _I, _VP, _VP, _I, _I, C.POINTER(DebugConfigC), _VP,
                          _I64, _VP]),
    "mi355_conv2d_ex": (_I, [_VP, _VP, _I, _FP, _FP, _VP, _I, _I, _I, _I, _I, _I, _I, _I, _VP, _VP, _I, _VP, _VP, _I, _I, C.POINTER(DebugConfigC), _VP,
                             _I64, _VP, C.POINTER(ConvExtrasC)]),
    "mi355_qkv_attention": (_I, [_VP, _VP, _I, _I, _I, _I, _I, _I, _VP, _I64, _VP]),
    "mi355_qkv_attention_vjp": (_I, [_VP, _VP, _VP, _I, _I, _I, _I, _I, _I, _VP, _I64, _VP]),
    "mi355_attn_block_fused": (_I, [_VP, _VP, _VP, _FP, _FP, _VP, _I, _I, _I, _I, _I, _I, C.POINTER(DebugConfigC), C.POINTER(C.c_int32), _VP, _I64, _VP]),
    "mi355_gn_affine": (_I, [_VP, _VP, _VP, _VP, _VP, _F, _VP, _VP, _VP, _VP, _VP, _I, C.POINTER(C.c_int32), _I, _I, _I, _I, _I, _VP]),
    "mi355_conv2d_gn": (_I, [_VP, _FP, _FP, _VP, _I, _I, _VP, _FP, _FP, _VP, _I, _I, _I, _I, _I, _I, _I, _I, _VP, _VP, _VP, _F, _VP, _VP, _I,
                             C.POINTER(DebugConfigC), C.POINTER(C.c_int32), _VP]),
    "mi355_affine_pool": (_I, [_VP, _VP, _VP, _I, _VP, _I, _I, _I, _I, _I, _VP]),
    "mi355_gn_silu_vjp": (_I, [_VP, _VP, _VP, _VP, _VP, _F, _I, _VP, _I, _VP, _VP, _I, _I, _I, _I, _I, _I, _I, _VP]),
    "mi355_grad_gather": (_I, [_VP, _VP, _I, _I, _I, _I, _I, _I, _I, _I, _I, _I, _F, _I, _VP]),
    "mi355_conv2d_vjp": (_I, [_FP, _VP, _VP, _VP, _VP, _I, _I, _I, _I, _I, _I, _I, _I, _I, _I, _I, _I, _I, C.POINTER(DebugConfigC), C.POINTER(C.c_int32), _VP,
                              _I64, _VP]),
}

_lock = threading.Lock()
_lib = None


def build(force: bool = False) -> str:
    if force:
        subprocess.run(["make", "-C", CSRC, "clean"], check=True, capture_output=True)
    r = subprocess.run(["make", "-C", CSRC, "-j8"], capture_output=True, text=True)
    if r.returncode != 0:
        raise MI355BackendError("building libmi355_sampler.so failed:\n" + r.stdout[-4000:] + r.stderr[-4000:])
    return LIB_PATH


def lib():
    global _lib
    with _lock:
        if _lib is not None:
            return _lib
        if not os.path.exists(LIB_PATH):
            raise MI355BackendError(
                f"{LIB_PATH} is missing: build it with `make -C {CSRC}` (or `python -c 'import __graft_entry__ as g; g.build()'`). "
                "This package has no CPU or PyTorch fallback.")
        import torch

        try:
            L = C.CDLL(LIB_PATH)
        except OSError as e:
            raise MI355BackendError(f"cannot load {LIB_PATH}: {e}") from e
        for name, (res, args) in SIGNATURES.items():
            fn = getattr(L, name)
            fn.restype = res
            fn.argtypes = args
        _lib = L
        return L


def check(rc: int, what: str = ""):
    if rc is not None and rc < 0:
        msg = lib().mi355_last_error().decode("utf-8", "replace")
        raise MI355BackendError(f"{what or 'libmi355_sampler'} failed ({rc}): {msg}")
# ... 35 lines not shown
```

### image-inpainting-and-super-resolution-using-diffusion-models-and-conditional-flow-matching_amd/mi355/ops.py

```python
from __future__ import annotations

import ctypes as C

import torch

from . import _lib
from ._lib import MI355BackendError, check


def _stream():
    return C.c_void_p(torch.cuda.current_stream().cuda_stream)


def _req(t: torch.Tensor, name: str, dtype=torch.float32):
    if not isinstance(t, torch.Tensor):
        raise TypeError(f"{name} must be a tensor")
    if not t.is_cuda:
        raise MI355BackendError(f"{name} is on {t.device}: the MI355X HIP backend needs device tensors (no CPU fallback)")
    if t.dtype != dtype:
        raise TypeError(f"{name} must be {dtype}, got {t.dtype}")
    if not t.is_contiguous():
        raise ValueError(f"{name} must be contiguous")
    return C.c_void_p(t.data_ptr())

# ... 155 lines not shown
    def quantize_u8(self, x):
        out = torch.empty(x.shape, device=x.device, dtype=torch.uint8)
        check(_lib.lib().mi355_quantize_u8(_req(x, "x"), _req(out, "out", torch.uint8), x.numel(), _stream()))
        return out

    def to_unit_range(self, x):
        out = torch.empty_like(x)
        check(_lib.lib().mi355_to_unit_range(_req(x, "x"), _req(out, "out"), x.numel(), _stream()))
        return out

    def randn(self, shape, device, seed, offset=0):
        out = torch.empty(shape, device=device, dtype=torch.float32)
        check(_lib.lib().mi355_randn(_req(out, "out"), int(seed), int(offset), out.numel(), _stream()))
        return out

    def rk_combine(self, out, y0, ks, coeffs):
        assert len(ks) == len(coeffs) <= 7
        arr = (C.c_float * 7)(*([float(c) for c in coeffs] + [0.0] * (7 - len(coeffs))))
        kp = [_req(k, "k") for k in ks] + [None] * (7 - len(ks))
        check(_lib.lib().mi355_rk_combine(_req(out, "out"), _req(y0, "y0") if y0 is not None else None, *kp, arr, len(ks), out.numel(),
                                          _stream()))
        return out

    def rk_stage(self, out, y0, ks, coeffs, copy_out=None, u8_out=None):
        if not 1 <= len(ks) == len(coeffs) <= 4:
            raise ValueError("rk_stage takes 1 to 4 stage derivatives, one coefficient each")
        _same(out, y0, "out", "y0")
        for k in ks:
            _same(out, k, "out", "k")
        if copy_out is not None:
            _same(out, copy_out, "out", "copy_out")
        if u8_out is not None:
            _same(out, u8_out, "out", "u8_out")
        arr = (C.c_float * 4)(*([float(c) for c in coeffs] + [0.0] * (4 - len(coeffs))))
        kp = (C.c_void_p * 4)(*([_req(k, "k") for k in ks] + [None] * (4 - len(ks))))
        check(_lib.lib().mi355_rk_stage(_req(out, "out"), _req(y0, "y0"), kp, arr, len(ks), out.numel(),
                                        _req(copy_out, "copy_out") if copy_out is not None else None,
                                        _req(u8_out, "u8_out", torch.uint8) if u8_out is not None else None, _stream()), "mi355_rk_stage")
        return out

    @staticmethod
    def _cfg_w(w, B):
        if isinstance(w, torch.Tensor) and w.dim() > 0:
            if tuple(w.shape) != (B,):
                raise ValueError(f"a per-image guidance scale must have shape ({B},), got {tuple(w.shape)}")
            w = w.to(torch.float32).contiguous()
            return 0.0, _req(w, "w"), w
        return float(w), None, None

    def cfg_stage(self, out, y0, ks, coeffs, w, dup=False, copy_out=None, u8_out=None):
        if not 1 <= len(ks) == len(coeffs) <= 4:
            raise ValueError("cfg_stage takes 1 to 4 stage derivatives, one coefficient each")
        B2 = ks[0].shape[0]
        if B2 % 2:
            raise ValueError("the derivatives hold the conditional and the unconditional evaluation: an even leading size")
        B = B2 // 2
        half = (B,) + tuple(ks[0].shape[1:])
        for k in ks:
            _same(ks[0], k, "k", "k")
        if tuple(out.shape) != ((B2,) + half[1:] if dup else half):
            raise ValueError(f"out must be {(B2,) + half[1:] if dup else half}, got {tuple(out.shape)}")
        for t, nm in ((y0, "y0"), (copy_out, "copy_out"), (u8_out, "u8_out")):
            if t is not None and tuple(t.shape) != half and not (nm == "y0" and dup and tuple(t.shape) == tuple(out.shape)):
                raise ValueError(f"{nm} must be {half}, got {tuple(t.shape)}")
        n = ks[0].numel() // 2
        wf, wp, keep = self._cfg_w(w, B)
        arr = (C.c_float * 4)(*([float(c) for c in coeffs] + [0.0] * (4 - len(coeffs))))
        kp = (C.c_void_p * 4)(*([_req(k, "k") for k in ks] + [None] * (4 - len(ks))))
        check(_lib.lib().mi355_cfg_stage(_req(out, "out"), _req(y0, "y0") if y0 is not None else None, kp, arr, len(ks), n, wf, wp,
                                         n // B if B else 1, int(bool(dup)), _req(copy_out, "copy_out") if copy_out is not None else None,
                                         _req(u8_out, "u8_out", torch.uint8) if u8_out is not None else None, _stream()), "mi355_cfg_stage")
        return out

    def cfg_combine(self, v2, w, out=None):
        if out is None:
            out = torch.empty((v2.shape[0] // 2,) + tuple(v2.shape[1:]), device=v2.device, dtype=torch.float32)
        return self.cfg_stage(out, None, [v2], [1.0], w)

    def ddpm_cfg_step_(self, x2, eps2, z, w, c_recip, c_recipm1, coef1, coef2, sigma, philox=None):
        _same(x2, eps2, "x2", "eps2")
        B = x2.shape[0] // 2
        if x2.shape[0] % 2:
            raise ValueError("x2 holds the state twice: an even leading size")
        n = x2.numel() // 2
        if z is not None and z.numel() != n:
            raise ValueError("z must have the B-image state's size")
        wf, wp, keep = self._cfg_w(w, B)
        seed, off = philox if philox else (0, 0)
        check(_lib.lib().mi355_ddpm_cfg_step(_req(x2, "x2"), _req(eps2, "eps2"), _req(z, "z") if z is not None else None, wf, wp, n // B if B else 1,
                                             c_recip, c_recipm1, coef1, coef2, sigma, int(philox is not None and z is None), seed, off, n, _stream()),
              "mi355_ddpm_cfg_step")
        return x2

    def ddim_cfg_step_(self, x2, eps2, w, c_recip, c_recipm1, acp_prev):
        _same(x2, eps2, "x2", "eps2")
        if x2.shape[0] % 2:
            raise ValueError("x2 holds the state twice: an even leading size")
        B = x2.shape[0] // 2
        n = x2.numel() // 2
        wf, wp, keep = self._cfg_w(w, B)
        check(_lib.lib().mi355_ddim_cfg_step(_req(x2, "x2"), _req(eps2, "eps2"), wf, wp, n // B if B else 1, c_recip, c_recipm1, acp_prev, n, _stream()),
              "mi355_ddim_cfg_step")
        return x2

    def rk_sqnorm(self, acc, a, sub=None, b=None, b2=None, atol=1.0, rtol=0.0):
        check(_lib.lib().mi355_rk_sqnorm(_req(a, "a"), _req(sub, "sub") if sub is not None else None, _req(b, "b") if b is not None else None,
                                         _req(b2, "b2") if b2 is not None else None, float(atol), float(rtol), a.numel(),
                                         _req(acc, "acc", torch.float64), _stream()))
        return acc

    def rk_interp(self, out, y0, y1, ymid, f0, f1, dt, x):
        check(_lib.lib().mi355_rk_interp(_req(out, "out"), _req(y0, "y0"), _req(y1, "y1"), _req(ymid, "ymid"), _req(f0, "f0"), _req(f1, "f1"),
                                         float(dt), float(x), out.numel(), _stream()))
        return out

    def conv2d(self, x, weight, bias=None, stride=1, resample=0, gn=None, gn_silu=False, dtype=_lib.MI355_F32, x1=None, emb=None,
               res=None, res_mode=1, debug=None, info=None):
        B, Cin, H, W = x.shape
        Co, Ci, k, _ = weight.shape
        Cin1 = 0 if x1 is None else x1.shape[1]
        assert Ci == Cin + Cin1
        if x1 is not None and (x1.shape[0] != B or x1.shape[2:] != x.shape[2:]):
            raise ValueError("x1 must match x in batch and spatial size")
        Hc = H * 2 if resample == 2 else (H // 2 if resample == 3 else H)
        Wc = W * 2 if resample == 2 else (W // 2 if resample == 3 else W)
        Ho = (Hc + 2 * (k // 2) - k) // stride + 1
        Wo = (Wc + 2 * (k // 2) - k) // stride + 1
        if emb is not None and emb.shape != (B, Co):
            raise ValueError("emb must be [B, Co]")
        if res is not None:
            want = (B, Co, Ho, Wo) if res_mode == 1 else (B, Co, Ho // 2, Wo // 2)
            if tuple(res.shape) != want:
                raise ValueError(f"res must be {want}")
        y = torch.empty(B, Co, Ho, Wo, device=x.device, dtype=torch.float32)
        L = _lib.lib()
        wsb = L.mi355_op_workspace_bytes(B, max(Ci, Co), max(H * W, Ho * Wo))
        ws = torch.empty(wsb, device=x.device, dtype=torch.uint8)
        w = weight.detach().to("cpu", torch.float32).contiguous()
        b = bias.detach().to("cpu", torch.float32).contiguous() if bias is not None else None
        fp = C.POINTER(C.c_float)
        args = (_req(x, "x"), _req(x1, "x1") if x1 is not None else None, Cin1, C.cast(w.data_ptr(), fp),
                C.cast(b.data_ptr(), fp) if b is not None else None, _req(y, "y"), B, Cin, H, W, Co, k, stride, resample,
                _req(gn[0], "gamma") if gn else None, _req(gn[1], "beta") if gn else None, int(gn_silu),
                _req(emb, "emb") if emb is not None else None, _req(res, "res") if res is not None else None, int(res_mode),
                dtype, C.byref(debug if debug is not None else _lib.debug_config()), C.c_void_p(ws.data_ptr()), wsb, _stream())
        if info is None:
            check(L.mi355_conv2d(*args), "mi355_conv2d")
        else:
            ex = _lib.ConvExtrasC()
            check(L.mi355_conv2d_ex(*args, C.byref(ex)), "mi355_conv2d_ex")
            info.update(kernel=ex.route[0], form=ex.route[1], tile_m=ex.route[2], tile_n=ex.route[3])
        return y

    def conv2d_ex(self, x, weight, bias, dtype=_lib.MI355_F32, skip=None, sites=(), film=None, debug=None):
        B, Cin, H, W = x.shape
        Co, Ci, k, _ = weight.shape
        assert Ci == Cin and k == 3 and len(sites) <= 2
        y = torch.empty(B, Co, H, W, device=x.device, dtype=torch.float32)
        L = _lib.lib()
        wsb = L.mi355_op_workspace_bytes(B, max(Ci, Co), H * W)
        ws = torch.empty(wsb, device=x.device, dtype=torch.uint8)
        w = weight.detach().to("cpu", torch.float32).contiguous()
        b = bias.detach().to("cpu", torch.float32).contiguous() if bias is not None else None
        fp = C.POINTER(C.c_float)
        ex = _lib.ConvExtrasC()
        keep = []
        if skip is not None:
            xs0, xs1, w1, b1 = skip
            w1c = w1.detach().to("cpu", torch.float32).reshape(Co, -1).contiguous()
            b1c = b1.detach().to("cpu", torch.float32).contiguous() if b1 is not None else None
            keep += [w1c, b1c]
            ex.skip_x0 = _req(xs0, "skip_x0"); ex.skip_c0 = xs0.shape[1]
            if xs1 is not None:
                ex.skip_x1 = _req(xs1, "skip_x1"); ex.skip_c1 = xs1.shape[1]
            ex.skip_w_host = w1c.data_ptr()
            ex.skip_bias_host = b1c.data_ptr() if b1c is not None else None
        acts = []
        for i, st in enumerate(sites):
            a = torch.full((B, st["ctotal"], H, W), float("nan"), device=x.device, dtype=torch.float32)
            acts.append(a)
            ex.act_out[i] = _req(a, "act_out"); ex.act_gamma[i] = _req(st["gamma"], "gamma"); ex.act_beta[i] = _req(st["beta"], "beta")
            ex.act_ctotal[i] = st["ctotal"]; ex.act_coff[i] = st["coff"]; ex.act_silu[i] = int(st.get("silu", True))
        if film is not None:
            ex.act_film = _req(film, "film")
        check(L.mi355_conv2d_ex(_req(x, "x"), None, 0, C.cast(w.data_ptr(), fp), C.cast(b.data_ptr(), fp) if b is not None else None, _req(y, "y"),
                                B, Cin, H, W, Co, 3, 1, 0, None, None, 0, None, None, 1, dtype,
                                C.byref(debug if debug is not None else _lib.debug_config()), C.c_void_p(ws.data_ptr()), wsb, _stream(), C.byref(ex)),
              "mi355_conv2d_ex")
        return y, [a if (ex.act_done >> i) & 1 else None for i, a in enumerate(acts)], bool(ex.skip_done)

    def qkv_attention(self, qkv, heads, new_order=False, dtype=_lib.MI355_F32):
        B, width, T = qkv.shape
        ch = width // (3 * heads)
        out = torch.empty(B, heads * ch, T, device=qkv.device, dtype=torch.float32)
        L = _lib.lib()
        wsb = L.mi355_op_workspace_bytes(B, width, T)
        ws = torch.empty(wsb, device=qkv.device, dtype=torch.uint8)
        check(L.mi355_qkv_attention(_req(qkv, "qkv"), _req(out, "out"), B, heads, ch, T, int(new_order), dtype,
                                    C.c_void_p(ws.data_ptr()), wsb, _stream()), "mi355_qkv_attention")
        return out

    def qkv_attention_vjp(self, qkv, grad_out, heads, new_order=False, dtype=_lib.MI355_F32, ws_fill=None):
        B, width, T = qkv.shape
        ch = width // (3 * heads)
        if tuple(grad_out.shape) != (B, heads * ch, T):
            raise ValueError(f"grad_out must be {(B, heads * ch, T)}, got {tuple(grad_out.shape)}")
        gq = torch.empty_like(qkv)
        L = _lib.lib()
        wsb = L.mi355_op_workspace_bytes(B, width, T)
        ws = torch.empty(wsb, device=qkv.device, dtype=torch.uint8) if ws_fill is None else \
            torch.full((wsb,), int(ws_fill), device=qkv.device, dtype=torch.uint8)
        check(L.mi355_qkv_attention_vjp(_req(qkv, "qkv"), _req(grad_out, "grad_out"), _req(gq, "grad_qkv"), B, heads, ch, T, int(new_order),
                                        dtype, C.c_void_p(ws.data_ptr()), wsb, _stream()), "mi355_qkv_attention_vjp")
        return gq

    def attn_block_fused(self, x, a, b, weight, bias, heads, new_order=False, dtype=_lib.MI355_F32, debug=None):
        B, Cc, T = x.shape
        if tuple(a.shape) != (B, Cc) or tuple(b.shape) != (B, Cc):
            raise ValueError(f"a and b must be {(B, Cc)}")
        w = weight.detach().to("cpu", torch.float32).reshape(weight.shape[0], -1).contiguous()
        bh = bias.detach().to("cpu", torch.float32).contiguous()
        if tuple(w.shape) != (3 * Cc, Cc) or tuple(bh.shape) != (3 * Cc,):
            raise ValueError(f"weight must be {(3 * Cc, Cc)} and bias {(3 * Cc,)}")
        out = torch.empty(B, Cc, T, device=x.device, dtype=torch.float32)
        L = _lib.lib()
        wsb = L.mi355_op_workspace_bytes(B, 3 * Cc, T)
        ws = torch.empty(wsb, device=x.device, dtype=torch.uint8)
        fp = C.POINTER(C.c_float)
        form = (C.c_int32 * 3)(-1, -1, -1)
        check(L.mi355_attn_block_fused(_req(x, "x"), _req(a, "a"), _req(b, "b"), C.cast(w.data_ptr(), fp), C.cast(bh.data_ptr(), fp), _req(out, "out"),
                                       B, Cc, T, heads, int(new_order), dtype, C.byref(debug if debug is not None else _lib.debug_config()),
                                       form, C.c_void_p(ws.data_ptr()), wsb, _stream()), "mi355_attn_block_fused")
        return out, (("image", form[1]) if form[0] == 1 else ("persistent", form[1], form[2]))

    def gn_affine(self, x, gamma, beta, x1=None, film=None, eps=1e-5, dtype=_lib.MI355_F32, apply=None, stats=True):
        B, C0 = x.shape[:2]
        C1 = 0 if x1 is None else x1.shape[1]
        hw = x[0, 0].numel()
        if x1 is not None and (x1.shape[0] != B or x1[0, 0].numel() != hw):
            raise ValueError("x1 must match x in batch and spatial size")
        Cc = C0 + C1
        if tuple(gamma.shape) != (Cc,) or tuple(beta.shape) != (Cc,) or (film is not None and tuple(film.shape) != (B, 2 * Cc)):
            raise ValueError("gamma / beta must be [C0 + C1], film [B, 2 (C0 + C1)]")
        if apply not in (None, "affine", "silu"):
            raise ValueError("apply must be None, 'affine' or 'silu'")
        dev = x.device
        a = torch.full((B, Cc), float("nan"), device=dev)
        b = torch.full((B, Cc), float("nan"), device=dev)
        mean = torch.full((B, 32), float("nan"), device=dev) if stats else None
        rstd = torch.full((B, 32), float("nan"), device=dev) if stats else None
        y = torch.full((B, Cc) + tuple(x.shape[2:]), float("nan"), device=dev) if apply else None
        form = C.c_int32(-1)
        check(_lib.lib().mi355_gn_affine(_req(x, "x"), _req(x1, "x1") if x1 is not None else None, _req(gamma, "gamma"), _req(beta, "beta"),
                                         _req(film, "film") if film is not None else None, float(eps), _req(a, "a"), _req(b, "b"),
                                         _req(mean, "mean") if stats else None, _req(rstd, "rstd") if stats else None,
                                         _req(y, "y") if apply else None, int(apply == "silu"), C.byref(form), B, C0, C1, hw, dtype, _stream()),
              "mi355_gn_affine")
        return dict(a=a, b=b, mean=mean, rstd=rstd, y=y, form=form.value)

    def conv2d_gn(self, x, weight, bias, gamma, beta, x1=None, weight1=None, bias1=None, film=None, eps=1e-5, stride=1, resample=0,
                  dtype=_lib.MI355_F32, debug=None):
        B, Cin, H, W = x.shape
        Co, Ci, k, _ = weight.shape
        assert Ci == Cin
        Co1 = 0
        if x1 is not None:
            Co1, Ci1, k1, _ = weight1.shape
            assert Ci1 == x1.shape[1] and k1 == k and x1.shape[0] == B and x1.shape[2:] == x.shape[2:]
        Hc, Wc = (H * 2, W * 2) if resample == 2 else (H, W)
        Ho = (Hc + 2 * (k // 2) - k) // stride + 1
        Wo = (Wc + 2 * (k // 2) - k) // stride + 1
        Cc = Co + Co1
        if tuple(gamma.shape) != (Cc,) or tuple(beta.shape) != (Cc,) or (film is not None and tuple(film.shape) != (B, 2 * Cc)):
            raise ValueError("gamma / beta must be [Co + Co1], film [B, 2 (Co + Co1)]")
        dev = x.device
        y = torch.full((B, Co, Ho, Wo), float("nan"), device=dev)
        y1 = torch.full((B, Co1, Ho, Wo), float("nan"), device=dev) if x1 is not None else None
        a = torch.full((B, Cc), float("nan"), device=dev)
        b = torch.full((B, Cc), float("nan"), device=dev)
        fp = C.POINTER(C.c_float)
        host = lambda t: t.detach().to("cpu", torch.float32).contiguous() if t is not None else None
        w0, b0, w1, b1 = host(weight), host(bias), host(weight1), host(bias1)
        hp = lambda t: C.cast(t.data_ptr(), fp) if t is not None else None
        info = (C.c_int32 * 6)()
        check(_lib.lib().mi355_conv2d_gn(_req(x, "x"), hp(w0), hp(b0), _req(y, "y"), Cin, Co,
                                         _req(x1, "x1") if x1 is not None else None, hp(w1), hp(b1), _req(y1, "y1") if x1 is not None else None,
                                         x1.shape[1] if x1 is not None else 0, Co1, B, H, W, k, stride, resample, _req(gamma, "gamma"),
                                         _req(beta, "beta"), _req(film, "film") if film is not None else None, float(eps), _req(a, "a"), _req(b, "b"),
                                         dtype, C.byref(debug if debug is not None else _lib.debug_config()), info, _stream()), "mi355_conv2d_gn")
        return dict(y=y, y1=y1, a=a, b=b, kernel=info[0], slots=info[1], form=info[2], kernel1=info[3], slots1=info[4], form1=info[5])

    def affine_pool(self, x, a=None, b=None, silu=False, dtype=_lib.MI355_F32):
        B, Cc, H, W = x.shape
        if (a is None) != (b is None) or (a is not None and (tuple(a.shape) != (B, Cc) or tuple(b.shape) != (B, Cc))):
            raise ValueError("a and b must both be [B, C] or both None")
        out = torch.full((B, Cc, H // 2, W // 2), float("nan"), device=x.device)
        check(_lib.lib().mi355_affine_pool(_req(x, "x"), _req(a, "a") if a is not None else None, _req(b, "b") if b is not None else None,
                                           int(bool(silu)), _req(out, "out"), B, Cc, H, W, dtype, _stream()), "mi355_affine_pool")
        return out

    def gn_silu_vjp(self, x, du, gamma, beta, x1=None, film=None, eps=1e-5, silu=True, du_stride=None, g0=None, g1=None,
                    dtype=_lib.MI355_F32):
        B, C0 = x.shape[:2]
        C1 = 0 if x1 is None else x1.shape[1]
        hw = x[0, 0].numel()
        Cc = C0 + C1
        if tuple(du.shape[:2]) != (B, Cc) or du[0, 0].numel() != hw:
            raise ValueError("du must be [B, C0 + C1, *] with x's spatial size")
        if tuple(gamma.shape) != (Cc,) or tuple(beta.shape) != (Cc,) or (film is not None and tuple(film.shape) != (B, 2 * Cc)):
            raise ValueError("gamma / beta must be [C0 + C1], film [B, 2 (C0 + C1)]")
        acc0, acc1 = g0 is not None, g1 is not None
        if acc0:
            _same(g0, x, "g0", "x")
        if acc1:
            _same(g1, x1, "g1", "x1")
        g0 = g0 if acc0 else torch.full_like(x, float("nan"))
        g1 = None if x1 is None else (g1 if acc1 else torch.full_like(x1, float("nan")))
        check(_lib.lib().mi355_gn_silu_vjp(_req(x, "x"), _req(x1, "x1") if x1 is not None else None, _req(gamma, "gamma"), _req(beta, "beta"),
                                           _req(film, "film") if film is not None else None, float(eps), int(bool(silu)), _req(du, "du"),
                                           int(du_stride or Cc), _req(g0, "g0"), _req(g1, "g1") if g1 is not None else None, int(acc0), int(acc1),
                                           B, C0, C1, hw, dtype, _stream()), "mi355_gn_silu_vjp")
        return g0, g1

    def grad_gather(self, src, shape, mode, coff=0, scale=1.0, dst=None, dtype=_lib.MI355_F32):
        B, Cs, Hs, Ws = src.shape
        Cd, Hd, Wd = shape
        acc = dst is not None
        if acc and tuple(dst.shape) != (B, Cd, Hd, Wd):
            raise ValueError("dst must be [B, Cd, Hd, Wd]")
        out = dst if acc else torch.full((B, Cd, Hd, Wd), float("nan"), device=src.device)
        check(_lib.lib().mi355_grad_gather(_req(src, "src"), _req(out, "dst"), B, Cd, Hd, Wd, Hs, Ws, Cs, int(coff), int(mode), int(acc),
                                           float(scale), dtype, _stream()), "mi355_grad_gather")
        return out

    def conv2d_vjp(self, weight, grad_out, c0, c1=0, hw=None, mode=0, g_channels=None, g0=None, g1=None, raw=False, dtype=_lib.MI355_F32,
                   debug=None, ws_fill=None, info=None):
        Co, Ci, k, _ = weight.shape
        B = grad_out.shape[0]
        h, w = hw if hw is not None else tuple(grad_out.shape[2:])
        Ho, Wo = ((h - 1) // 2 + 1, (w - 1) // 2 + 1) if mode == 1 else ((2 * h, 2 * w) if mode == 2 else (h, w))
        if tuple(grad_out.shape) != (B, Co, Ho, Wo):
# ... 38 lines not shown
```

### include/mi355_sampler.h

```cpp
#ifndef MI355_SAMPLER_H
#define MI355_SAMPLER_H

#include <stddef.h>
#include <stdint.h>

#ifdef __cplusplus
extern "C" {
#endif

#define MI355_OK 0
#define MI355_ERR_ARG (-1)
#define MI355_ERR_SHAPE (-2)
#define MI355_ERR_HIP (-3)
#define MI355_ERR_UNSUPPORTED (-4)
#define MI355_ERR_TIMEOUT (-5)

#define MI355_F32 0
#define MI355_BF16 1
#define MI355_BF16X2 2
#define MI355_F16 3

int mi355_version(void);
const char* mi355_last_error(void);

// ... 90 lines not shown
  int32_t kind, ks, cin, cout, h, w;
  int32_t tile_m, tile_n;
  float ms;
  double flops;
  double bytes;
} mi355_op_profile;
int mi355_unet_profile(mi355_unet* net, const float* x, int x_channels, const float* cond, int cond_channels, const float* t,
                       float* out, int batch, void* workspace, int64_t workspace_bytes, void* stream,
                       mi355_op_profile* recs, int cap);


int mi355_cfm_euler_sample(mi355_unet* net, float* x, int x_channels, const float* cond, int cond_channels, int cond_drift,
                           const float* t_span_host, int n_t, float* traj, uint8_t* u8_out, int batch,
                           void* workspace, int64_t workspace_bytes, void* stream);

int mi355_cfm_euler_sample_labels(mi355_unet* net, float* x, int x_channels, const float* cond, int cond_channels, int cond_drift,
                                  const int32_t* labels, const float* t_span_host, int n_t, float* traj, uint8_t* u8_out, int batch,
                                  void* workspace, int64_t workspace_bytes, void* stream);

int64_t mi355_cfm_rk_workspace_bytes(const mi355_unet* net, int batch, int stages);
int mi355_cfm_rk_sample(mi355_unet* net, float* x, int x_channels, const float* cond, int cond_channels, const int32_t* labels,
                        const float* t_span_host, int n_t, int stages, const float* a_host, const float* b_host, const float* c_host,
                        float* traj, uint8_t* u8_out, int batch, void* workspace, int64_t workspace_bytes, void* stream);

int mi355_sf2m_euler_sample(mi355_unet* drift, mi355_unet* score, float* x, int channels, const int32_t* labels, const float* t_grid_host,
                            int n_steps, float sigma, int reverse, const float* dW, uint64_t seed, const int32_t* out_step_host,
                            const float* out_w_host, int n_out, float* traj, int batch, void* drift_workspace, int64_t drift_workspace_bytes,
                            void* score_workspace, int64_t score_workspace_bytes, void* stream);

typedef struct mi355_ddpm_tables {
  int32_t Ns;
  const float* sqrt_recip_alphas_cumprod;
  const float* sqrt_recipm1_alphas_cumprod;
  const float* posterior_mean_coef1;
  const float* posterior_mean_coef2;
  const float* posterior_log_variance_clipped;
  const float* sqrt_alphas_cumprod;
  const float* sqrt_one_minus_alphas_cumprod;
  const float* recip_sqrt_m1_alphas_cumprod;
  const float* alphas_cumprod_prev;
} mi355_ddpm_tables;

#define MI355_DDPM_PRIOR 0
#define MI355_DDPM_AMORTIZED 1
#define MI355_DDPM_REPLACEMENT 2
#define MI355_DDIM 3

typedef struct mi355_ddpm_options {
  int32_t mode;
  int32_t n_corrector;
  float delta;
  float tmin, tmax;
  float start_fraction;
  int32_t noise_condition;
  float pad_value;
  float none_value;
  int32_t cond_is_none;
  uint64_t seed;
} mi355_ddpm_options;

int mi355_ddpm_sample(mi355_unet* net, float* x, int channels, const float* cond, const mi355_ddpm_tables* tables,
                      const mi355_ddpm_options* opt, const float* noise, int64_t n_noise_draws, int batch,
                      void* workspace, int64_t workspace_bytes, void* stream);

int64_t mi355_cfg_workspace_bytes(const mi355_unet* net, int batch, int stages);
int mi355_cfm_cfg_sample(mi355_unet* net, float* x, int x_channels, const float* cond, int cond_channels, float none_value, const int32_t* labels,
                         int null_label, float w, const float* w_dev, const float* t_span_host, int n_t, int stages, const float* a_host,
                         const float* b_host, const float* c_host, float* traj, uint8_t* u8_out, int batch, void* workspace, int64_t workspace_bytes,
                         void* stream);
int64_t mi355_ddpm_cfg_workspace_bytes(const mi355_unet* net, int batch);
int mi355_ddpm_cfg_sample(mi355_unet* net, float* x, int channels, const float* cond, const int32_t* labels, int null_label, float w, const float* w_dev,
                          const mi355_ddpm_tables* tables, const mi355_ddpm_options* opt, const float* noise, int64_t n_noise_draws, int batch,
                          void* workspace, int64_t workspace_bytes, void* stream);

int64_t mi355_cfm_recon_workspace_bytes(const mi355_unet* net, int batch, int h_low, int w_low);
int mi355_cfm_recon_sample(mi355_unet* net, float* x, int channels, const int32_t* labels, const float* t_span_host, int n_t, const float* y, int mode,
                           float pad_value, int h_low, int w_low, const float* scales_host, int replace, int final_paste, const float* z, uint64_t seed,
                           float* traj, uint8_t* u8_out, float* loss_out, int batch, void* workspace, int64_t workspace_bytes, void* stream);


int mi355_timestep_embedding(const float* t, int batch, int dim, float max_period, float* out, void* stream);

int mi355_groupnorm(const float* x, const float* gamma, const float* beta, float* y, int batch, int channels, int hw,
                    int groups, float eps, int silu, void* stream);

int mi355_euler_step(float* x, const float* v, float dt, int64_t n, void* stream);

int mi355_sde_euler_step(float* x, const float* a, const float* b, float ca, float cb, float dt, const float* g, float g_scalar, const float* dW,
                         int use_philox, uint64_t seed, uint64_t offset, float* out, float w, int64_t n, void* stream);

int mi355_ddpm_step(float* x, const float* eps, const float* z, float c_recip, float c_recipm1, float coef1, float coef2,
                    float sigma, int use_philox, uint64_t seed, uint64_t offset, int64_t n, void* stream);

int mi355_corrector_step(float* x, const float* eps, const float* z, float c_recip, float c_recipm1, float recip_sqrt_m1,
                         float dt, float delta, int use_philox, uint64_t seed, uint64_t offset, int64_t n, void* stream);

int mi355_ddim_step(float* x, const float* eps, float c_recip, float c_recipm1, float acp_prev, int64_t n, void* stream);

int mi355_replace_mask(float* x, const float* cond, const float* z, float pad_value, int noisy, float sa, float sb,
                       int use_philox, uint64_t seed, uint64_t offset, int64_t n, void* stream);

int mi355_guidance_seed(const float* x, const float* eps, const float* cond, float c_recip, float c_recipm1, int mode, float pad_value,
                        int64_t elems_per_sample, float* g_eps, float* g_x, int64_t n, void* stream);
int mi355_guidance_update(float* x, const float* g_x, const float* vjp, float scale, int apply, float* update, int64_t n, void* stream);

int mi355_lowres_seed(const float* x, const float* eps, const float* y_low, float c_recip, float c_recipm1, int batch, int channels, int h, int w,
                      int h_low, int w_low, float* resid, float* g_eps, float* g_x, float* loss, void* stream);

int mi355_clip(float* x, float lo, float hi, int64_t n, void* stream);
int mi355_ema_update(float* target, const float* source, float decay, float one_minus_decay, int64_t n, void* stream);
int mi355_mse_per_sample(const float* a, const float* b, float* out, int batch, int64_t elems_per_sample, void* stream);
int mi355_lincomb_per_sample(float* out, const float* x, const float* y, const float* a, const float* b, int batch,
                             int64_t elems_per_sample, void* stream);
int mi355_resize_bilinear(const float* in, float* out, int64_t planes, int h_in, int w_in, int h_out, int w_out, void* stream);
int mi355_paint_patch(const float* images, const int32_t* top, const int32_t* left, int patch_size, float pad_value, int outpaint,
                      float* out, int batch, int channels, int h, int w, void* stream);
int mi355_quantize_u8(const float* x, uint8_t* out, int64_t n, void* stream);
int mi355_to_unit_range(const float* x, float* out, int64_t n, void* stream);
int mi355_randn(float* out, uint64_t seed, uint64_t offset, int64_t n, void* stream);

int mi355_rk_combine(float* out, const float* y0, const float* k0, const float* k1, const float* k2, const float* k3, const float* k4,
                     const float* k5, const float* k6, const float* coeff_host, int nk, int64_t n, void* stream);
int mi355_rk_stage(float* out, const float* y0, const float* const k[4], const float* coeff_host, int nk, int64_t n, float* copy_out,
                   uint8_t* u8_out, void* stream);
int mi355_cfg_stage(float* out, const float* y0, const float* const k[4], const float* coeff_host, int nk, int64_t n, float w, const float* w_dev,
                    int64_t elems_per_image, int dup, float* copy_out, uint8_t* u8_out, void* stream);
int mi355_ddpm_cfg_step(float* x, const float* eps, const float* z, float w, const float* w_dev, int64_t elems_per_image, float c_recip, float c_recipm1,
                        float coef1, float coef2, float sigma, int use_philox, uint64_t seed, uint64_t offset, int64_t n, void* stream);
int mi355_ddim_cfg_step(float* x, const float* eps, float w, const float* w_dev, int64_t elems_per_image, float c_recip, float c_recipm1, float acp_prev,
                        int64_t n, void* stream);
int mi355_rk_sqnorm(const float* a, const float* sub, const float* b, const float* b2, float atol, float rtol, int64_t n, double* out,
                    void* stream);
int mi355_rk_interp(float* out, const float* y0, const float* y1, const float* y_mid, const float* f0, const float* f1, float dt, float x,
                    int64_t n, void* stream);

int64_t mi355_box_probe_workspace_bytes(void);
int mi355_box_probe(int reps, void* workspace, int64_t workspace_bytes, void* stream, float* us_per_launch, float* clock_mhz, float* tflop);
int64_t mi355_box_probe_hbm_workspace_bytes(void);
int mi355_box_probe_hbm(int reps, void* workspace, int64_t workspace_bytes, void* stream, float* us_per_launch, float* gbytes);

int64_t mi355_op_workspace_bytes(int batch, int max_channels, int hw);
int mi355_conv2d(const float* x, const float* x1, int cin1, const float* w_host, const float* bias_host, float* y, int batch, int cin,
                 int h, int w, int cout, int ksize, int stride, int resample, const float* gn_gamma, const float* gn_beta, int gn_silu,
                 const float* emb, const float* res, int res_mode, int dtype, const mi355_debug_config* debug, void* workspace,
                 int64_t workspace_bytes, void* stream);
typedef struct mi355_conv_extras {
  const float* skip_x0; const float* skip_x1; int32_t skip_c0, skip_c1;
  const float* skip_w_host; const float* skip_bias_host;
  float* act_out[2]; const float* act_gamma[2]; const float* act_beta[2];
  int32_t act_ctotal[2], act_coff[2], act_silu[2];
  const float* act_film;
  int32_t act_done, skip_done;
  int32_t route[4];
} mi355_conv_extras;
int mi355_conv2d_ex(const float* x, const float* x1, int cin1, const float* w_host, const float* bias_host, float* y, int batch, int cin,
                    int h, int w, int cout, int ksize, int stride, int resample, const float* gn_gamma, const float* gn_beta, int gn_silu,
                    const float* emb, const float* res, int res_mode, int dtype, const mi355_debug_config* debug, void* workspace,
                    int64_t workspace_bytes, void* stream, mi355_conv_extras* extras);
int mi355_qkv_attention(const float* qkv, float* out, int batch, int heads, int head_channels, int length, int new_order,
                        int dtype, void* workspace, int64_t workspace_bytes, void* stream);
int mi355_qkv_attention_vjp(const float* qkv, const float* grad_out, float* grad_qkv, int batch, int heads, int head_channels, int length,
                            int new_order, int dtype, void* workspace, int64_t workspace_bytes, void* stream);

int mi355_attn_block_fused(const float* x, const float* a, const float* b, const float* w_host, const float* bias_host, float* out, int batch,
                           int channels, int length, int heads, int new_order, int dtype, const mi355_debug_config* debug, int32_t form[3],
                           void* workspace, int64_t workspace_bytes, void* stream);

int mi355_gn_affine(const float* x, const float* x1, const float* gamma, const float* beta, const float* film, float eps, float* a, float* b,
                    float* mean, float* rstd, float* y, int y_silu, int32_t* form, int batch, int c0, int c1, int hw, int dtype, void* stream);
int mi355_conv2d_gn(const float* x0, const float* w0_host, const float* bias0_host, float* y0, int cin0, int cout0, const float* x1,
                    const float* w1_host, const float* bias1_host, float* y1, int cin1, int cout1, int batch, int h, int w, int ksize, int stride,
                    int resample, const float* gamma, const float* beta, const float* film, float eps, float* a, float* b, int dtype,
                    const mi355_debug_config* debug, int32_t info[6], void* stream);
int mi355_affine_pool(const float* x, const float* a, const float* b, int silu, float* out, int batch, int channels, int h, int w, int dtype,
                      void* stream);
int mi355_gn_silu_vjp(const float* x0, const float* x1, const float* gamma, const float* beta, const float* film, float eps, int silu,
                      const float* du, int du_stride, float* g0, float* g1, int acc0, int acc1, int batch, int c0, int c1, int hw, int dtype,
                      void* stream);
int mi355_grad_gather(const float* src, float* dst, int batch, int cd, int hd, int wd, int hs, int ws, int src_channels, int src_coff, int mode,
                      int accumulate, float scale, int dtype, void* stream);
int mi355_conv2d_vjp(const float* w_host, const float* grad_out, float* g0, float* g1, float* du_raw, int acc0, int acc1, int batch, int cout,
                     int cin, int c0, int c1, int h, int w, int ksize, int mode, int g_channels, int dtype, const mi355_debug_config* debug,
                     int32_t route[4], void* workspace, int64_t workspace_bytes, void* stream);

#ifdef __cplusplus
}
#endif
#endif
```

Measured before the change: 1408.

## Carry the 1x1 skip convolution inside the persistent warp-specialized 3x3 conv kernel

Extends the persistent warp-specialized 3x3 conv kernel with a SKIP variant. It streams extra weight and skip-input tiles, interleaved between the main row pairs, so the residual block's 1x1 skip convolution accumulates into the same output tile. The default conv_ws knob now enables this path, and the U-Net planner carries the skip conv for more blocks (the 16x16+ resolutions with Cout not a multiple of 256). The goal is to remove separate skip-conv launches and the round trip of the skip result through memory. In exchange the producer/consumer schedule and LDS use become more complex, and the load across the pipeline can become uneven. The diff also adds a grid cap knob and statistics plumbing in the C API and Python bindings.

```diff
diff --git a/image-inpainting-and-super-resolution-using-diffusion-models-and-conditional-flow-matching_amd/csrc/capi.hip b/image-inpainting-and-super-resolution-using-diffusion-models-and-conditional-flow-matching_amd/csrc/capi.hip
--- a/image-inpainting-and-super-resolution-using-diffusion-models-and-conditional-flow-matching_amd/csrc/capi.hip
+++ b/image-inpainting-and-super-resolution-using-diffusion-models-and-conditional-flow-matching_amd/csrc/capi.hip
@@ -17,7 +17,7 @@
 void mi355_debug_defaults(mi355_debug_config* c) {
   if (!c) return;
   std::memset(c, 0, sizeof(*c));
-  c->conv_ws = 1; c->conv_small = 15; c->conv_min_wgs = 512; c->conv_stagger = 0; c->conv_ablate = 0; c->conv_spin_limit = 1 << 22;
+  c->conv_ws = 3; c->conv_small = 15; c->conv_min_wgs = 512; c->conv_stagger = 0; c->conv_ablate = 0; c->conv_spin_limit = 1 << 22;
   c->conv_time_reps = 0; c->gn_apply_max_hw = 64; c->gn_fuse = 1; c->l2_warm = 1; c->attn_fused = 1; c->gn_epilogue = 7; c->conv_pp = 109; c->conv_edge = 15;
 }
 int mi355_unet_status(mi355_unet* net, int clear) {
diff --git a/image-inpainting-and-super-resolution-using-diffusion-models-and-conditional-flow-matching_amd/csrc/conv_igemm.hip b/image-inpainting-and-super-resolution-using-diffusion-models-and-conditional-flow-matching_amd/csrc/conv_igemm.hip
--- a/image-inpainting-and-super-resolution-using-diffusion-models-and-conditional-flow-matching_amd/csrc/conv_igemm.hip
+++ b/image-inpainting-and-super-resolution-using-diffusion-models-and-conditional-flow-matching_amd/csrc/conv_igemm.hip
@@ -787,7 +787,8 @@
   const bool gn_ok = d.gn_stats && d.out_mode == OUT_NHWC && g.G == 1 && d.Cout % g.BN == 0 && d.Cout % 4 == 0;
   const bool has_pro = d.pro_a != nullptr;
   const bool up_ok = d.mode == CONV_UP2 && d.w_up2 && !d.wsplit && a.res_mode == RES_NONE;
-  const int pc = fskip ? -1 : pp_config(K.conv_pp, d.ks, g.G, g.bn_pack, d.out_mode, g.stride, a.nchunks, has_pro, d.pro_silu != 0, d.N, g.Ho, g.Wo, d.Cout, up_ok);
+  const int pc_alone = pp_config(K.conv_pp, d.ks, g.G, g.bn_pack, d.out_mode, g.stride, a.nchunks, has_pro, d.pro_silu != 0, d.N, g.Ho, g.Wo, d.Cout, up_ok);
+  const int pc = fskip ? -1 : pc_alone;
   if (pc == 2) {
     r->kernel = CONV_K_PP; r->form = 2; r->w_up2 = 1;
     r->geom.BM = 256; r->geom.BN = 256; r->geom.lds_bytes = pp::D<0>::lds_bytes(false);
@@ -805,8 +806,9 @@
     if (!r->act_done && gn_ok && slots <= d.gn_slots_cap) r->gn_slots = slots;
     return 0;
   }
-  if (!fskip && ws_eligible(K.conv_ws, d.ks, g.BM, g.BN, g.G, g.bn_pack, d.out_mode, g.stride, a.nchunks, d.N, g.Ho, g.Wo, d.Cout)) {
-    r->kernel = CONV_K_WS;
+  if (ws_eligible(K.conv_ws, d.ks, g.BM, g.BN, g.G, g.bn_pack, d.out_mode, g.stride, a.nchunks, d.N, g.Ho, g.Wo, d.Cout) &&
+      (!fskip || (pc_alone < 0 && ws_skip_eligible(K.conv_ws, a, d.mode, d.act_out != nullptr, d.wsplit != 0, CH)))) {
+    r->kernel = CONV_K_WS; r->skip = fskip ? 1 : 0;
     r->geom.BM = 256; r->geom.lds_bytes = ws::LDS_BYTES;
     const int slots = 2 * ((g.Wo + ws::VW - 1) / ws::VW) * ((g.Ho + ws::TH - 1) / ws::TH);
     if (gn_ok && slots <= d.gn_slots_cap) r->gn_slots = slots;
@@ -856,7 +858,7 @@
   }
   int rc;
   if (r.kernel == CONV_K_PP) rc = dispatch_dtype(d.dtype, [&](auto t) { return launch_pp<decltype(t)>(a, r.form, stream); });
-  else if (r.kernel == CONV_K_WS) rc = dispatch_dtype(d.dtype, [&](auto t) { return launch_ws<decltype(t)>(a, stream); });
+  else if (r.kernel == CONV_K_WS) rc = dispatch_dtype(d.dtype, [&](auto t) { return launch_ws<decltype(t)>(a, (d.knobs ? d.knobs : &mi355_default_debug())->conv_ws >> 8, stream); });
   else if (r.kernel == CONV_K_SMALL) {
     if (r.act_done & 1) {
       a.act_stride = d.act_stride ? d.act_stride : d.Cout; a.act_coff = d.act_coff; a.act_cpg = d.act_cpg ? d.act_cpg : d.Cout / 32;
diff --git a/image-inpainting-and-super-resolution-using-diffusion-models-and-conditional-flow-matching_amd/csrc/conv_ws.inc.h b/image-inpainting-and-super-resolution-using-diffusion-models-and-conditional-flow-matching_amd/csrc/conv_ws.inc.h
--- a/image-inpainting-and-super-resolution-using-diffusion-models-and-conditional-flow-matching_amd/csrc/conv_ws.inc.h
+++ b/image-inpainting-and-super-resolution-using-diffusion-models-and-conditional-flow-matching_amd/csrc/conv_ws.inc.h
@@ -17,6 +17,8 @@
 constexpr int CBUF = BN * 4;
 constexpr int NPLANES = 3, NWBUF = 4;
 constexpr size_t LDS_BYTES = NPLANES * (size_t)PLANE + NWBUF * 3 * (size_t)WTILE + 2 * CBUF + 64;
+__host__ __device__ constexpr int skip_pair_first(int rp, int nrp, int np) { return rp * np / nrp; }
+__host__ __device__ constexpr int skip_pairs(int rp, int nrp, int np) { return skip_pair_first(rp + 1, nrp, np) - skip_pair_first(rp, nrp, np); }
 }
 
 typedef __bf16 bf16x2_t __attribute__((ext_vector_type(2)));
@@ -53,8 +55,9 @@
   return __builtin_bit_cast(u32x4, o);
 }
 
-template <typename T, int PRO>
+template <typename T, int PRO, bool SKIP = false>
 __global__ void __launch_bounds__(512, 2) conv3x3_ws_kernel(ConvKArgs p, int n_mt, int n_nt) {
+  static_assert(!SKIP || PRO != 0, "the carried skip conv rides in the prologue forms");
   using namespace ws;
   using E = Elem<T>;
   constexpr int V = E::VEC, CHUNK = E::CHUNK, ESZ = sizeof(T);
@@ -70,6 +73,9 @@
   const bool loader = wave8 < 4;
   const int tpi = p.tiles_x * p.tiles_y;
   const int ngr = p.nchunks * 3;
+  const int nsk = SKIP ? (p.SC0 + p.SC1) / CHUNK : 0;
+  const int nsp = (nsk + 1) >> 1, nrp = ngr >> 1;
+  const int wtiles = p.nchunks * 9 + nsk;
   const int ntp = ((n_mt + 7) / 8) * 8 * n_nt;
   auto decode = [&](int t, int& mt, int& nt) {
     const int per = 8 * n_nt, blk = t / per, r = t - blk * per;
@@ -430,8 +436,21 @@
     };
 
     int wl_t = t_first, wl_row = 0, wl_nt, wl_buf = 0;
-    { int mt; decode(wl_t, mt, wl_nt); }
+    int wl_k = 0, wl_s = 0, wl_n = 0;
+    int spix[4] = {-1, -1, -1, -1};
+    const uint32_t sfq16 = (uint32_t)(((lane & 3) ^ ((lane >> 3) & 3)) * 16);
+    auto skip_setup = [&](int mt) {
+      int n0, y0, x0;
+      origin(mt, n0, y0, x0);
+#pragma unroll
+      for (int i = 0; i < 4; ++i) {
+        const int y = y0 + 4 * i + wave8, x = x0 + (lane >> 2);
+        spix[i] = (y < p.Ho && x < p.Wo) ? (n0 * p.Ho + y) * p.Wo + x : -1;
+      }
+    };
+    { int mt; decode(wl_t, mt, wl_nt); if constexpr (SKIP) skip_setup(mt); }
     auto dma_w = [&]() {
+      if constexpr (!SKIP) {
       const uint32_t so = ((uint32_t)wl_nt * p.nchunks * 9 + (uint32_t)wl_row * 3) * WTILE;
       if constexpr (!(WS_ABLATE & 8)) {
         char* dst = wbuf + wl_buf * (3 * WTILE) + wave8 * 1024;
@@ -444,6 +463,43 @@
         wl_row = 0;
         wl_t = next_valid(wl_t);
         if (wl_t < ntp) { int mt; decode(wl_t, mt, wl_nt); }
+      }
+      } else {
+      char* dst = wbuf + wl_buf * (3 * WTILE) + wave8 * 1024;
+      if (wl_k == 0) {
+        const uint32_t so = ((uint32_t)wl_nt * wtiles + (uint32_t)(wl_row * 3)) * WTILE;
+#pragma unroll
+        for (int i = 0; i < WIT; ++i)
+          __builtin_amdgcn_raw_ptr_buffer_load_lds(rsw, (__attribute__((address_space(3))) void*)(dst + i * 4096), 16, woff[i], so, 0, 0);
+      } else {
+        const int sidx = __builtin_amdgcn_readfirstlane(wl_s);
+        const uint32_t so = ((uint32_t)wl_nt * wtiles + (uint32_t)(p.nchunks * 9 + sidx)) * WTILE;
+        const bool real = sidx < nsk;
+#pragma unroll
+        for (int i = 0; i < 2; ++i)
+          __builtin_amdgcn_raw_ptr_buffer_load_lds(rsw, (__attribute__((address_space(3))) void*)(dst + i * 4096), 16, real ? woff[i] : p.wbytes, so, 0, 0);
+        const int cb = sidx * CHUNK;
+        const bool first = cb < p.SC0;
+        const uint32_t pixb = (uint32_t)((first ? p.SC0 : p.SC1) * ESZ), oob = first ? p.skbytes0 : p.skbytes1;
+        const __amdgpu_buffer_rsrc_t rsk = __builtin_amdgcn_make_buffer_rsrc(const_cast<void*>(first || !p.sk1 ? p.sk0 : p.sk1), 0, oob, 0x00020000);
+        const uint32_t cso = (uint32_t)((first ? cb : cb - p.SC0) * ESZ);
+#pragma unroll
+        for (int i = 0; i < 4; ++i) {
+          const uint32_t vo = (spix[i] >= 0 && real) ? (uint32_t)spix[i] * pixb + sfq16 : oob;
+          __builtin_amdgcn_raw_ptr_buffer_load_lds(rsk, (__attribute__((address_space(3))) void*)(dst + WTILE + i * 4096), 16, vo, cso, 0, 0);
+        }
+        ++wl_s;
+      }
+      wl_buf = wl_buf == NWBUF - 1 ? 0 : wl_buf + 1;
+      if (wl_k == 0) wl_n = (wl_row & 1) ? 2 * skip_pairs(wl_row >> 1, nrp, nsp) : 0;
+      if (wl_k++ == wl_n) {
+        wl_k = 0;
+        if (++wl_row == ngr) {
+          wl_row = 0; wl_s = 0;
+          wl_t = next_valid(wl_t);
+          if (wl_t < ntp) { int mt; decode(wl_t, mt, wl_nt); skip_setup(mt); }
+        }
+      }
       }
     };
     auto wait_landed = [&]() {
@@ -498,6 +554,7 @@
       const int t_next = next_valid(t);
       auto body = [&](int c) {
         bool nx_ok = true;
+        int row = 3 * c;
         auto tail = [&]() {
           dma_w();
           STAMP(3)
@@ -507,6 +564,20 @@
           ++R;
           acquire_free();
           STAMP(4)
+          if constexpr (SKIP) {
+            if (row & 1) {
+              const int n = 2 * skip_pairs(row >> 1, nrp, nsp);
+              for (int j = 0; j < n; ++j) {
+                dma_w();
+                asm volatile("" ::: "memory");
+                __builtin_amdgcn_s_waitcnt(6 | (7 << 4) | (0 << 8));
+                bump(c_prod + wave8);
+                ++R;
+                acquire_free();
+              }
+            }
+            ++row;
+          }
         };
         cinit_load(t_next < ntp ? t_next : t);
         commit_frag(IC<4>(), plane, vmask_cm); issue_frag(IC<4>());
@@ -573,32 +644,47 @@
     uint32_t rowc = 0;
     uint32_t pq0 = 0, pq1 = 0, pq2 = 0, pq3 = 0;
     const bool gate512 = p.N > 0;
-    auto advance_row = [&]() {
+    auto advance_row = [&](bool main_row) __attribute__((always_inline)) {
       int bstep = 3 * WTILE, astep = AROWB;
       if (sel == NWBUF - 1) { sel = 0; bstep = -(NWBUF - 1) * 3 * WTILE; } else ++sel;
-      if (++ky == 3) {
-        ky = 0;
-        if (plane == NPLANES - 1) { plane = 0; astep = -(NPLANES - 1) * PLANE - 2 * AROWB; } else { ++plane; astep = PLANE - 2 * AROWB; }
-      }
-#pragma unroll
-      for (int kx = 0; kx < 3; ++kx) a_cur[kx] += astep;
+      if (main_row) {
+        if (++ky == 3) {
+          ky = 0;
+          if (plane == NPLANES - 1) { plane = 0; astep = -(NPLANES - 1) * PLANE - 2 * AROWB; } else { ++plane; astep = PLANE - 2 * AROWB; }
+        }
+#pragma unroll
+        for (int kx = 0; kx < 3; ++kx) a_cur[kx] += astep;
+      }
       b_cur += bstep;
     };
-    auto read_a = [&](auto bufc, auto halfc, auto kxc) {
+    const int sa_delta = WTILE + (wm * 128 - wn * 64) * 64;
+    auto read_sa = [&](auto halfc) __attribute__((always_inline)) {
+      constexpr int half = decltype(halfc)::value;
+#pragma unroll
+      for (int j = 0; j < 4; ++j) af[half][j] = *reinterpret_cast<const u32x4*>(wbuf + b_cur + sa_delta + (half * 4 + j) * 1024);
+    };
+    auto read_next = [&](bool next_skip) __attribute__((always_inline)) {
+      const int base = next_skip ? NPLANES * PLANE + b_cur + sa_delta : a_cur[0];
+      const int pitch = next_skip ? 1024 : AROWB;
+#pragma unroll
+      for (int j = 0; j < 4; ++j) af[0][j] = *reinterpret_cast<const u32x4*>(smem + base + j * pitch);
+    };
+    auto read_a = [&](auto bufc, auto halfc, auto kxc) __attribute__((always_inline)) {
       constexpr int buf = decltype(bufc)::value, half = decltype(halfc)::value, kx = decltype(kxc)::value;
       if constexpr (WS_ABLATE & 4) return;
       if constexpr (WS_ABLATE & 512) { if (gate512) return; }
 #pragma unroll
       for (int j = 0; j < 4; ++j) af[buf][j] = *reinterpret_cast<const u32x4*>(pbuf + a_cur[kx] + (half * 4 + j) * AROWB);
     };
-    auto read_b = [&](auto bufc, auto kxc) {
+    auto read_b = [&](auto bufc, auto kxc) __attribute__((always_inline)) {
       constexpr int buf = decltype(bufc)::value, kx = decltype(kxc)::value;
       if constexpr (WS_ABLATE & 4) return;
       if constexpr (WS_ABLATE & 512) { if (gate512) return; }
 #pragma unroll
       for (int ni = 0; ni < NI; ++ni) bf[buf][ni] = *reinterpret_cast<const u32x4*>(wbuf + b_cur + kx * WTILE + ni * 1024);
     };
-    auto step = [&](auto Rc, auto sc, auto zeroc, bool more_rows) {
+    auto step = [&](auto Rc, auto sc, auto zeroc, bool more_rows, auto nkc, bool next_skip = false) __attribute__((always_inline)) {
+      constexpr int nk = decltype(nkc)::value;
       constexpr int R = decltype(Rc)::value, s = decltype(sc)::value;
       constexpr bool ZERO = decltype(zeroc)::value != 0;
       constexpr int half = s & 1, kx = s >> 1, bpar = (R + kx) & 1;
@@ -613,8 +699,8 @@
           if constexpr (!(WS_ABLATE & 2048)) release_acquire(c_cons + wave, c_prod, rowc + 2u, pq0, pq1, pq2, pq3);
           ++rowc;
           STAMP(5)
-          advance_row();
-          read_a(IC<0>(), IC<0>(), IC<0>());
+          advance_row(true);
+          if constexpr (nk == 3) read_next(next_skip); else read_a(IC<0>(), IC<0>(), IC<0>());
           read_b(IC<(R + 1) & 1>(), IC<0>());
         }
       }
@@ -641,6 +727,26 @@
 #pragma unroll
           for (int ni = 0; ni < NI; ++ni) acc[half * 4 + j][ni] = cin[ni];
       }
+      __builtin_amdgcn_sched_barrier(0);
+    };
+
+    auto sstep = [&](auto Qc, auto halfc, bool more_rows, auto nkc, bool next_skip) __attribute__((always_inline)) {
+      constexpr int Q = decltype(Qc)::value, half = decltype(halfc)::value, nk = decltype(nkc)::value;
+      if constexpr (half == 0) {
+        read_sa(IC<1>());
+        poll_issue(c_prod, pq0, pq1, pq2, pq3);
+      } else if (more_rows) {
+        release_acquire(c_cons + wave, c_prod, rowc + 2u, pq0, pq1, pq2, pq3);
+        ++rowc;
+        advance_row(false);
+        if constexpr (nk == 1) read_sa(IC<0>()); else read_next(next_skip);
+        read_b(IC<Q ^ 1>(), IC<0>());
+      }
+      __builtin_amdgcn_sched_barrier(0);
+#pragma unroll
+      for (int j = 0; j < 4; ++j)
+#pragma unroll
+        for (int ni = 0; ni < NI; ++ni) mma16(acc[half * 4 + j][ni], bf[Q][ni], af[half][j], T());
       __builtin_amdgcn_sched_barrier(0);
     };
 
@@ -656,13 +762,22 @@
       const int co_w = nt * BN + wn * 64 + 4 * lq;
       for (int r = 0; r < ngr; r += 2) {
         const bool last_pair = r + 2 >= ngr;
-        if (r == 0) { read_cinit(); step(IC<0>(), IC<0>(), IC<1>(), true); step(IC<0>(), IC<1>(), IC<1>(), true); }
-        else { step(IC<0>(), IC<0>(), IC<0>(), true); step(IC<0>(), IC<1>(), IC<0>(), true); }
-        step(IC<0>(), IC<2>(), IC<0>(), true); step(IC<0>(), IC<3>(), IC<0>(), true);
-        step(IC<0>(), IC<4>(), IC<0>(), true); step(IC<0>(), IC<5>(), IC<0>(), true);
-        step(IC<1>(), IC<0>(), IC<0>(), true); step(IC<1>(), IC<1>(), IC<0>(), true);
-        step(IC<1>(), IC<2>(), IC<0>(), true); step(IC<1>(), IC<3>(), IC<0>(), true);
-        step(IC<1>(), IC<4>(), IC<0>(), true); step(IC<1>(), IC<5>(), IC<0>(), !last_pair);
+        if (r == 0) { read_cinit(); step(IC<0>(), IC<0>(), IC<1>(), true, IC<0>()); step(IC<0>(), IC<1>(), IC<1>(), true, IC<0>()); }
+        else { step(IC<0>(), IC<0>(), IC<0>(), true, IC<0>()); step(IC<0>(), IC<1>(), IC<0>(), true, IC<0>()); }
+        step(IC<0>(), IC<2>(), IC<0>(), true, IC<0>()); step(IC<0>(), IC<3>(), IC<0>(), true, IC<0>());
+        step(IC<0>(), IC<4>(), IC<0>(), true, IC<0>()); step(IC<0>(), IC<5>(), IC<0>(), true, IC<0>());
+        step(IC<1>(), IC<0>(), IC<0>(), true, IC<0>()); step(IC<1>(), IC<1>(), IC<0>(), true, IC<0>());
+        step(IC<1>(), IC<2>(), IC<0>(), true, IC<0>()); step(IC<1>(), IC<3>(), IC<0>(), true, IC<0>());
+        if constexpr (!SKIP) { step(IC<1>(), IC<4>(), IC<0>(), true, IC<0>()); step(IC<1>(), IC<5>(), IC<0>(), !last_pair, IC<0>()); }
+        else {
+          const int k = skip_pairs(r >> 1, nrp, nsp);
+          step(IC<1>(), IC<4>(), IC<0>(), true, IC<0>()); step(IC<1>(), IC<5>(), IC<0>(), true, IC<3>(), k > 0);
+          for (int q = 0; q < k; ++q) {
+            const bool more = !(last_pair && q + 1 == k);
+            sstep(IC<0>(), IC<0>(), true, IC<1>(), true); sstep(IC<0>(), IC<1>(), true, IC<1>(), true);
+            sstep(IC<1>(), IC<0>(), true, IC<3>(), true); sstep(IC<1>(), IC<1>(), more, IC<3>(), q + 1 < k);
+          }
+        }
       }
       if (t_next < ntp) bump(c_cons + wave);
       if constexpr ((WS_ABLATE & 256) != 0) {
@@ -760,7 +875,7 @@
       if (t_next < ntp) {
         if constexpr (!(WS_ABLATE & 2048)) wait_ge_prod(c_prod, rowc + 2u);
         ++rowc;
-        advance_row();
+        advance_row(!SKIP);
         read_a(IC<0>(), IC<0>(), IC<0>());
         read_b(IC<0>(), IC<0>());
       }
@@ -776,15 +891,20 @@
   return ncu;
 }
 static bool ws_eligible(int enabled, int ks, int BM, int BN, int G, int bn_pack, int out_mode, int stride, int nchunks, int N, int Ho, int Wo, int Cout) {
-  if (!enabled || ks != 3 || BM != 128 || BN != 128 || G != 1 || bn_pack != 128 || out_mode != OUT_NHWC) return false;
+  if (!(enabled & 1) || ks != 3 || BM != 128 || BN != 128 || G != 1 || bn_pack != 128 || out_mode != OUT_NHWC) return false;
   if (stride != 1 || nchunks < 2 || (nchunks & 1)) return false;
   if (Wo < ws::VW || Ho < ws::TH) return false;
   const int n_mt = N * ((Wo + ws::VW - 1) / ws::VW) * ((Ho + ws::TH - 1) / ws::TH), n_nt = (Cout + 127) / 128;
-  return n_mt * n_nt >= ws_num_cus();
+  return (enabled & 4) || n_mt * n_nt >= ws_num_cus();
 }
+static bool ws_skip_eligible(int enabled, const ConvKArgs& a, int mode, bool fused_act, bool wsplit, int CH) {
+  if (!(enabled & 2) || !a.sk0 || !a.pro_a || wsplit || mode != CONV_UNIT || fused_act || a.res_mode != RES_NONE) return false;
+  if (a.SC0 <= 0 || a.SC0 % CH || a.SC1 % CH) return false;
+  return true;
+}
 
 template <typename T>
-int launch_ws(ConvKArgs a, hipStream_t s) {
+int launch_ws(ConvKArgs a, int grid_cap, hipStream_t s) {
   a.lvw = 4; a.lth = 4; a.PW = ws::PW; a.PH = ws::PH; a.NP = ws::NPX;
   a.tiles_x = (a.Wo + ws::VW - 1) / ws::VW; a.tiles_y = (a.Ho + ws::TH - 1) / ws::TH;
   const int n_mt = a.N * a.tiles_x * a.tiles_y, n_nt = (a.Cout + 127) / 128;
@@ -792,12 +912,17 @@
   using KernT = void (*)(ConvKArgs, int, int);
   KernT kern = !a.pro_a ? (KernT)conv3x3_ws_kernel<T, 0> : (a.pro_silu ? (KernT)conv3x3_ws_kernel<T, 2> : (KernT)conv3x3_ws_kernel<T, 1>);
   int rc;
+  if (a.sk0) {
+    kern = a.pro_silu ? (KernT)conv3x3_ws_kernel<T, 2, true> : (KernT)conv3x3_ws_kernel<T, 1, true>;
+    rc = a.pro_silu ? mi355_allow_big_lds(conv3x3_ws_kernel<T, 2, true>, "conv3x3 (persistent)") : mi355_allow_big_lds(conv3x3_ws_kernel<T, 1, true>, "conv3x3 (persistent)");
+  } else
   if (!a.pro_a) rc = mi355_allow_big_lds(conv3x3_ws_kernel<T, 0>, "conv3x3 (persistent)");
   else if (a.pro_silu) rc = mi355_allow_big_lds(conv3x3_ws_kernel<T, 2>, "conv3x3 (persistent)");
   else rc = mi355_allow_big_lds(conv3x3_ws_kernel<T, 1>, "conv3x3 (persistent)");
   if (rc) return rc;
   const int ntp = ((n_mt + 7) / 8) * 8 * n_nt;
-  const int grid = ntp < ncu ? ntp : ncu;
+  int grid = ntp < ncu ? ntp : ncu;
+  if (grid_cap > 0 && grid_cap < grid) grid = grid_cap;
   hipLaunchKernelGGL(kern, dim3(grid), dim3(512), ws::LDS_BYTES, s, a, n_mt, n_nt);
   return 0;
 }
diff --git a/image-inpainting-and-super-resolution-using-diffusion-models-and-conditional-flow-matching_amd/csrc/unet_engine.hip b/image-inpainting-and-super-resolution-using-diffusion-models-and-conditional-flow-matching_amd/csrc/unet_engine.hip
--- a/image-inpainting-and-super-resolution-using-diffusion-models-and-conditional-flow-matching_amd/csrc/unet_engine.hip
+++ b/image-inpainting-and-super-resolution-using-diffusion-models-and-conditional-flow-matching_amd/csrc/unet_engine.hip
@@ -242,28 +242,32 @@
       return -1;
     }
     const int skip_idx = cin != cout ? (int)net->ops.size() - 1 : -1;
+    auto carry_skip = [&](int out) {
+      if (out < 0 || skip_idx < 0 || net->ops[skip_idx].ks != 1 || cfg.differentiable || net->wsplit || cout % 128 != 0) return;
+      const int conv2_idx = (int)net->ops.size() - 1;
+      PlanOp& c2 = net->ops[conv2_idx];
+      const float* w3 = P(p + ".out_layers.3.weight", {cout, cout, 3, 3});
+      const float* w1 = P(p + ".skip_connection.weight", {cout, cin, 1, 1});
+      const float* b3 = P(p + ".out_layers.3.bias", {cout});
+      const float* b1 = P(p + ".skip_connection.bias", {cout});
+      c2.wf_off = alloc(conv_packed_weight_bytes_skip(dtype, cout, cout, cin));
+      c2.bf_off = alloc((size_t)cout * 4);
+      if (!dry && w3 && w1 && b3 && b1) {
+        conv_pack_weights_skip(dtype, w3, w1, cout, cout, cin, blob.data() + c2.wf_off);
+        float* bs = reinterpret_cast<float*>(blob.data() + c2.bf_off);
+        for (int i = 0; i < cout; ++i) bs[i] = b3[i] + b1[i];
+      }
+      c2.skip_op = skip_idx;
+      net->ops[skip_idx].carrier = conv2_idx;
+    };
     if (y2 >= 0) {
       const int out = add_conv(p + ".out_layers.3", y2, -1, cout, cout, 3, CONV_UNIT, false, 0, 0, -1, res, res_mode, OUT_NHWC);
-      if (out >= 0 && skip_idx >= 0 && net->ops[skip_idx].ks == 1 && !cfg.differentiable && !net->wsplit && cout % 128 == 0) {
-        const int conv2_idx = (int)net->ops.size() - 1;
-        PlanOp& c2 = net->ops[conv2_idx];
-        const float* w3 = P(p + ".out_layers.3.weight", {cout, cout, 3, 3});
-        const float* w1 = P(p + ".skip_connection.weight", {cout, cin, 1, 1});
-        const float* b3 = P(p + ".out_layers.3.bias", {cout});
-        const float* b1 = P(p + ".skip_connection.bias", {cout});
-        c2.wf_off = alloc(conv_packed_weight_bytes_skip(dtype, cout, cout, cin));
-        c2.bf_off = alloc((size_t)cout * 4);
-        if (!dry && w3 && w1 && b3 && b1) {
-          conv_pack_weights_skip(dtype, w3, w1, cout, cout, cin, blob.data() + c2.wf_off);
-          float* bs = reinterpret_cast<float*>(blob.data() + c2.bf_off);
-          for (int i = 0; i < cout; ++i) bs[i] = b3[i] + b1[i];
-        }
-        c2.skip_op = skip_idx;
-        net->ops[skip_idx].carrier = conv2_idx;
-      }
+      carry_skip(out);
       return out;
     }
-    return add_conv(p + ".out_layers.3", h1, -1, cout, cout, 3, CONV_UNIT, false, 1, 1, -1, res, res_mode, OUT_NHWC);
+    const int out = add_conv(p + ".out_layers.3", h1, -1, cout, cout, 3, CONV_UNIT, false, 1, 1, -1, res, res_mode, OUT_NHWC);
+    if (out >= 0 && T(h1).W >= 16 && T(h1).H >= 16 && cout % 256 != 0) carry_skip(out);
+    return out;
   }
 
   int attn_block(const std::string& p, int x, int C, int heads) {
diff --git a/image-inpainting-and-super-resolution-using-diffusion-models-and-conditional-flow-matching_amd/mi355/_lib.py b/image-inpainting-and-super-resolution-using-diffusion-models-and-conditional-flow-matching_amd/mi355/_lib.py
--- a/image-inpainting-and-super-resolution-using-diffusion-models-and-conditional-flow-matching_amd/mi355/_lib.py
+++ b/image-inpainting-and-super-resolution-using-diffusion-models-and-conditional-flow-matching_amd/mi355/_lib.py
@@ -60,7 +60,8 @@
                 ("skip_w_host", C.c_void_p), ("skip_bias_host", C.c_void_p),
                 ("act_out", C.c_void_p * 2), ("act_gamma", C.c_void_p * 2), ("act_beta", C.c_void_p * 2),
                 ("act_ctotal", C.c_int32 * 2), ("act_coff", C.c_int32 * 2), ("act_silu", C.c_int32 * 2),
-                ("act_film", C.c_void_p), ("act_done", C.c_int32), ("skip_done", C.c_int32), ("route", C.c_int32 * 4)]
+                ("act_film", C.c_void_p), ("act_done", C.c_int32), ("skip_done", C.c_int32), ("route", C.c_int32 * 4),
+                ("stat_gamma", C.c_void_p), ("stat_beta", C.c_void_p), ("stat_a", C.c_void_p), ("stat_b", C.c_void_p), ("stat_slots", C.c_int32)]
 
 
 class UNetStatsC(C.Structure):
diff --git a/image-inpainting-and-super-resolution-using-diffusion-models-and-conditional-flow-matching_amd/mi355/ops.py b/image-inpainting-and-super-resolution-using-diffusion-models-and-conditional-flow-matching_amd/mi355/ops.py
--- a/image-inpainting-and-super-resolution-using-diffusion-models-and-conditional-flow-matching_amd/mi355/ops.py
+++ b/image-inpainting-and-super-resolution-using-diffusion-models-and-conditional-flow-matching_amd/mi355/ops.py
@@ -331,7 +331,8 @@
             info.update(kernel=ex.route[0], form=ex.route[1], tile_m=ex.route[2], tile_n=ex.route[3])
         return y
 
-    def conv2d_ex(self, x, weight, bias, dtype=_lib.MI355_F32, skip=None, sites=(), film=None, debug=None):
+    def conv2d_ex(self, x, weight, bias, dtype=_lib.MI355_F32, skip=None, sites=(), film=None, debug=None, gn=None, gn_silu=False, emb=None,
+                  stats=None):
         B, Cin, H, W = x.shape
         Co, Ci, k, _ = weight.shape
         assert Ci == Cin and k == 3 and len(sites) <= 2
@@ -362,10 +363,22 @@
             ex.act_ctotal[i] = st["ctotal"]; ex.act_coff[i] = st["coff"]; ex.act_silu[i] = int(st.get("silu", True))
         if film is not None:
             ex.act_film = _req(film, "film")
+        if stats is not None:
+            one, zero = torch.ones(Co, device=x.device), torch.zeros(Co, device=x.device)
+            sa, sb = torch.full((B, Co), float("nan"), device=x.device), torch.full((B, Co), float("nan"), device=x.device)
+            keep += [one, zero]
+            ex.route[3] = 0x53544154
+            ex.stat_gamma = _req(one, "stat_gamma"); ex.stat_beta = _req(zero, "stat_beta"); ex.stat_a = _req(sa, "stat_a"); ex.stat_b = _req(sb, "stat_b")
+        if emb is not None and emb.shape != (B, Co):
+            raise ValueError("emb must be [B, Co]")
         check(L.mi355_conv2d_ex(_req(x, "x"), None, 0, C.cast(w.data_ptr(), fp), C.cast(b.data_ptr(), fp) if b is not None else None, _req(y, "y"),
-                                B, Cin, H, W, Co, 3, 1, 0, None, None, 0, None, None, 1, dtype,
+                                B, Cin, H, W, Co, 3, 1, 0, _req(gn[0], "gamma") if gn else None, _req(gn[1], "beta") if gn else None, int(gn_silu),
+                                _req(emb, "emb") if emb is not None else None, None, 1, dtype,
                                 C.byref(debug if debug is not None else _lib.debug_config()), C.c_void_p(ws.data_ptr()), wsb, _stream(), C.byref(ex)),
               "mi355_conv2d_ex")
+        if stats is not None:
+            stats.update(slots=ex.stat_slots, a=sa if ex.stat_slots > 0 else None, b=sb if ex.stat_slots > 0 else None,
+                         kernel=ex.route[0], tile_m=ex.route[2], tile_n=ex.route[3])
         return y, [a if (ex.act_done >> i) & 1 else None for i, a in enumerate(acts)], bool(ex.skip_done)
 
     def qkv_attention(self, qkv, heads, new_order=False, dtype=_lib.MI355_F32):
diff --git a/include/mi355_sampler.h b/include/mi355_sampler.h
--- a/include/mi355_sampler.h
+++ b/include/mi355_sampler.h
@@ -266,7 +266,10 @@
   const float* act_film;
   int32_t act_done, skip_done;
   int32_t route[4];
+  const float* stat_gamma; const float* stat_beta; float* stat_a; float* stat_b;
+  int32_t stat_slots;
 } mi355_conv_extras;
+#define MI355_CONV_EXTRAS_STATS 0x53544154
 int mi355_conv2d_ex(const float* x, const float* x1, int cin1, const float* w_host, const float* bias_host, float* y, int batch, int cin,
                     int h, int w, int cout, int ksize, int stride, int resample, const float* gn_gamma, const float* gn_beta, int gn_silu,
                     const float* emb, const float* res, int res_mode, int dtype, const mi355_debug_config* debug, void* workspace,
```

Result: faster. 1438, median of 6 (+2.2%).
